# nwihardjo/SpaghettiSearch

Hardware: AMD Instinct MI355X
Metric: pagerank_iters_per_sec (higher is better)
Workload: dtype f64

## Files before the change

### spaghettisearch_amd/csrc/ctx.hip

```cpp
#include "common.hpp"
#include <chrono>

#include <unordered_map>

namespace ss {

namespace {
struct Pool {
    std::mutex mu;
    std::multimap<std::pair<int, size_t>, void*> free_blocks;
    std::unordered_map<void*, std::pair<int, size_t>> live;
    size_t held = 0, limit = (size_t)64 << 30;
    double miss_ms = 0.0;
    uint64_t misses = 0;
    int contexts = 0;
};
Pool& pool() { static Pool* p = new Pool(); return *p; }
size_t size_class(size_t b) {
    if (b <= 4096) return 4096;
    size_t p2 = 4096;
    while (p2 < b) p2 <<= 1;
    if (p2 <= ((size_t)1 << 20)) return p2;
    const size_t step = p2 >> 4;
    return (b + step - 1) / step * step;
}
}

hipError_t pool_alloc(void** out, size_t bytes) {
    Pool& P = pool();
    const size_t cls = size_class(bytes);
    int dev = 0;
    (void)hipGetDevice(&dev);
    {
        std::lock_guard<std::mutex> lk(P.mu);
        auto it = P.free_blocks.find({dev, cls});
        if (it != P.free_blocks.end()) {
            *out = it->second;
            P.free_blocks.erase(it);
            P.held -= cls;
            P.live[*out] = {dev, cls};
            return hipSuccess;
        }
    }
    const auto tm0 = std::chrono::steady_clock::now();
    hipError_t e = hipMalloc(out, cls);
    {
        std::lock_guard<std::mutex> lk(P.mu);
        P.miss_ms += std::chrono::duration<double, std::milli>(std::chrono::steady_clock::now() - tm0).count();
        P.misses++;
    }
    if (e != hipSuccess) {
        (void)hipGetLastError();
        pool_trim();
        e = hipMalloc(out, cls);
    }
    if (e == hipSuccess) {
        std::lock_guard<std::mutex> lk(P.mu);
        P.live[*out] = {dev, cls};
    }
    return e;
}

static thread_local bool t_device_idle = false;

void pool_free_batch(void* const* blocks, size_t count) {
    if (!count) return;
    {
        int cur = 0;
        (void)hipGetDevice(&cur);
        if (device_wedged(cur)) return;
    }
    (void)hipDeviceSynchronize();
    t_device_idle = true;
    for (size_t i = 0; i < count; i++) pool_free(blocks[i]);
    t_device_idle = false;
}

void pool_free(void* p) {
    if (!p) return;
    Pool& P = pool();
    size_t cls = 0, limit = 0;
    int dev = 0;
    {
        std::lock_guard<std::mutex> lk(P.mu);
        auto it = P.live.find(p);
        if (it != P.live.end()) { dev = it->second.first; cls = it->second.second; P.live.erase(it); }
        limit = P.limit;
    }
    if (device_wedged(dev)) return;
    if (cls && cls <= limit / 2) {
        int cur = 0;
        (void)hipGetDevice(&cur);
        if (cur != dev || !t_device_idle) {
            if (cur != dev) (void)hipSetDevice(dev);
            (void)hipDeviceSynchronize();
            if (cur != dev) (void)hipSetDevice(cur);
        }
        std::vector<void*> evict;
        {
            std::lock_guard<std::mutex> lk(P.mu);
            while (P.held + cls > P.limit && !P.free_blocks.empty()) {
                auto last = std::prev(P.free_blocks.end());
                if (last->first.second <= cls) break;
                evict.push_back(last->second);
                P.held -= last->first.second;
                P.free_blocks.erase(last);
            }
            if (P.held + cls <= P.limit) {
                P.free_blocks.emplace(std::make_pair(dev, cls), p);
                P.held += cls;
                p = nullptr;
            }
        }
        for (void* q : evict) (void)hipFree(q);
        if (!p) return;
    }
    (void)hipFree(p);
}

void pool_stats(uint64_t* misses, double* miss_ms) {
    std::lock_guard<std::mutex> lk(pool().mu);
    *misses = pool().misses;
    *miss_ms = pool().miss_ms;
}
void pool_context_count(int delta) {
    bool last = false;
    {
        std::lock_guard<std::mutex> lk(pool().mu);
        pool().contexts += delta;
        last = delta < 0 && pool().contexts <= 0;
    }
    if (last) pool_trim();
}

void pool_trim() {
    Pool& P = pool();
    std::multimap<std::pair<int, size_t>, void*> take;
    {
        std::lock_guard<std::mutex> lk(P.mu);
        take.swap(P.free_blocks);
        P.held = 0;
    }
    for (auto& kv : take) (void)hipFree(kv.second);
}

void pool_set_limit(size_t bytes) {
    {
        std::lock_guard<std::mutex> lk(pool().mu);
        pool().limit = bytes;
    }
    pool_trim();
}

static std::mutex g_err_mu;
static std::string g_err;
void set_global_error(const std::string& msg) {
    std::lock_guard<std::mutex> lk(g_err_mu);
    g_err = msg;
}
}

extern "C" {

int32_t ss_abi_version(void) { return SS_ABI_VERSION; }

int32_t ss_init(int32_t device_id, ss_ctx** out) {
    if (!out) {
        ss::set_global_error("ss_init: out is NULL");
        return SS_ERR_INVALID;
    }
    *out = nullptr;
    int n_dev = 0;
    hipError_t e = hipGetDeviceCount(&n_dev);
    if (e != hipSuccess || n_dev <= 0) {
        ss::set_global_error(std::string("ss_init: no HIP device (") + hipGetErrorString(e) + ")");
        return SS_ERR_NO_DEVICE;
    }
    if (device_id < 0 || device_id >= n_dev) {
        ss::set_global_error("ss_init: device_id out of range");
        return SS_ERR_INVALID;
    }
    ss_ctx* ctx = new (std::nothrow) ss_ctx();
    if (!ctx) return SS_ERR_OOM;
    ctx->device = device_id;
    if ((e = hipSetDevice(device_id)) != hipSuccess) {
        ss::set_global_error(std::string("ss_init: hipSetDevice: ") + hipGetErrorString(e));
        delete ctx;
        return SS_ERR_NO_DEVICE;
    }
    hipDeviceProp_t prop;
    if ((e = hipGetDeviceProperties(&prop, device_id)) != hipSuccess) {
        ss::set_global_error(std::string("ss_init: hipGetDeviceProperties: ") + hipGetErrorString(e));
        delete ctx;
        return SS_ERR_NO_DEVICE;
    }
    if (std::strncmp(prop.gcnArchName, "gfx950", 6) != 0) {
        ss::set_global_error(std::string("ss_init: device is ") + prop.gcnArchName +
                             ", this library is built for gfx950 (MI355X) only");
        delete ctx;
        return SS_ERR_NO_DEVICE;
    }
    ctx->cu_count = prop.multiProcessorCount;
    ctx->total_mem = prop.totalGlobalMem;
    if ((e = hipStreamCreateWithFlags(&ctx->own_stream, hipStreamNonBlocking)) != hipSuccess) {
        ss::set_global_error(std::string("ss_init: hipStreamCreate: ") + hipGetErrorString(e));
        delete ctx;
        return SS_ERR_HIP;
    }
    ctx->stream = ctx->own_stream;
    int prio_lo = 0, prio_hi = 0;
    (void)hipDeviceGetStreamPriorityRange(&prio_lo, &prio_hi);
    if ((e = hipStreamCreateWithPriority(&ctx->comm_stream, hipStreamNonBlocking, prio_hi)) != hipSuccess) {
        ss::set_global_error(std::string("ss_init: hipStreamCreate (comm): ") + hipGetErrorString(e));
        (void)hipStreamDestroy(ctx->own_stream);
        delete ctx;
        return SS_ERR_HIP;
    }
    for (int k = 0; k < 3; k++)
        for (int j = 0; j < 2; j++)
            if ((e = hipEventCreate(&ctx->ev[k][j])) != hipSuccess) {
                ss::set_global_error(std::string("ss_init: hipEventCreate: ") + hipGetErrorString(e));
                delete ctx;
                return SS_ERR_HIP;
            }
    if ((e = hipHostMalloc(reinterpret_cast<void**>(&ctx->h_pin), ss_ctx::PIN_SCRATCH, hipHostMallocDefault)) != hipSuccess) {
        ss::set_global_error(std::string("ss_init: hipHostMalloc: ") + hipGetErrorString(e));
        delete ctx;
        return SS_ERR_HIP;
    }
    ss::pool_context_count(+1);
    *out = ctx;
    return SS_OK;
}

int32_t ss_shutdown(ss_ctx* ctx) {
    if (!ctx) return SS_ERR_INVALID;
    (void)hipSetDevice(ctx->device);
    const bool stuck = !ss::try_unwedge(ctx);
    (void)ss_comm_destroy(ctx);
    if (!stuck) (void)hipStreamSynchronize(ctx->stream);
    for (int k = 0; k < 3; k++)
        for (int j = 0; j < 2; j++)
            if (ctx->ev[k][j]) (void)hipEventDestroy(ctx->ev[k][j]);
    if (ctx->comm_stream && !stuck) { (void)hipStreamSynchronize(ctx->comm_stream); (void)hipStreamDestroy(ctx->comm_stream); }
    for (hipStream_t ws : ctx->wave_stream)
        if (ws && !stuck) { (void)hipStreamSynchronize(ws); (void)hipStreamDestroy(ws); }
    if (ctx->own_stream && !stuck) (void)hipStreamDestroy(ctx->own_stream);
    if (ctx->h_pin) (void)hipHostFree(ctx->h_pin);
    for (auto& b : ctx->pin_cache) (void)hipHostFree(b.p);
    delete ctx;
    ss::pool_context_count(-1);
    return SS_OK;
}

int32_t ss_set_stream(ss_ctx* ctx, void* hip_stream) {
    if (!ctx) return SS_ERR_INVALID;
    std::lock_guard<std::recursive_mutex> lk(ctx->mu);
    SS_HIP(ctx, hipStreamSynchronize(ctx->stream));
    ctx->stream = hip_stream ? reinterpret_cast<hipStream_t>(hip_stream) : ctx->own_stream;
    return SS_OK;
}

static const char* const k_option_names[] = {
    "comm.timeout_ms",
    "pr.force_narrow",
    "pr.wire_f32",
    "pr.narrow_wave",
    "pr.t_quad",
    "pr.blocks_per_cu",
    "mem.pool_mb",
    "pr.deal_snake",
    "pr.affine_lag",
    "pr.affine",
    "pr.items_per_wave",
    "pr.persistent",
    "pr.persistent_blocks",
    "pr.n_class_order",
    "pr.class_order",
    "pr.stagger",
    "pr.deal_global",
    "pr.share_zero_rows",
    "pr.item_turns",
    "graph.late_free",
    "pr.trace",
    "score.collect_pinned",
    "score.pipeline_slices",
    "score.timing",
    "score.trace",
    "pr.probe_hot",
    "pr.topic_blocks",
    "tfidf.blocks",
    "tfidf.bucket_shift",
    "tfidf.head_min_run",
    "tfidf.bucket_min",
    "score.wave",
    "score.wave_max_terms",
    "score.wave_min_list",
    "score.wave_share_pct",
    "score.wave_slice_target",
    "score.wave_big_pct",
    "score.wave_big_x100",
    "score.small",
    "score.small_max_batch",
    "score.small_batch",
    "score.small_cap",
    "score.pipeline",
    "score.grade_slices",
    "score.wave_small_x100",
    "score.exact_all",
    "score.slice_target",
    "score.separate_merge",
};

int32_t ss_set_option(ss_ctx* ctx, const char* name, int64_t value) {
    if (!ctx || !name) return SS_ERR_INVALID;
    std::lock_guard<std::recursive_mutex> lk(ctx->mu);
    for (const char* n : k_option_names)
        if (std::strcmp(n, name) == 0) {
            if (value == SS_OPTION_DEFAULT) ctx->options.erase(name);
            else ctx->options[name] = value;
            if (std::strcmp(name, "mem.pool_mb") == 0) ss::pool_set_limit(value == SS_OPTION_DEFAULT ? (size_t)64 << 30 : (size_t)std::max<int64_t>(0, value) << 20);
            return SS_OK;
        }
    return ctx->fail(SS_ERR_INVALID, "ss_set_option: unknown option '%s'", name);
}

int32_t ss_synchronize(ss_ctx* ctx) {
    if (!ctx) return SS_ERR_INVALID;
    std::lock_guard<std::recursive_mutex> lk(ctx->mu);
    SS_HIP(ctx, hipSetDevice(ctx->device));
    SS_TRY(ss::sync_bounded(ctx, ctx->stream, "ss_synchronize"));
    return SS_OK;
}

const char* ss_last_error(ss_ctx* ctx) {
    if (ctx) return ctx->last_error.c_str();
    static thread_local std::string tl;
    {
        std::lock_guard<std::mutex> lk(ss::g_err_mu);
        tl = ss::g_err;
    }
    return tl.c_str();
}

int32_t ss_last_kernel_ms(ss_ctx* ctx, int32_t kind, float* ms_out) {
    if (!ctx || !ms_out || kind < 0 || kind > 2) return SS_ERR_INVALID;
    std::lock_guard<std::recursive_mutex> lk(ctx->mu);
    if (!ctx->ev_valid[kind]) return ctx->fail(SS_ERR_STATE, "ss_last_kernel_ms: no timed call of kind %d yet", kind);
    SS_HIP(ctx, hipEventSynchronize(ctx->ev[kind][1]));
    SS_HIP(ctx, hipEventElapsedTime(ms_out, ctx->ev[kind][0], ctx->ev[kind][1]));
    return SS_OK;
}

}
```

### spaghettisearch_amd/csrc/pagerank.hip

```cpp
#include "pr_device.hpp"

#include <algorithm>
#include <chrono>
#include <cmath>
#include <memory>

namespace {

__global__ void k_pr_item_ranges(WorkItem* __restrict__ work, uint32_t n_items, const uint32_t* __restrict__ in_ptr) {
    const uint32_t i = blockIdx.x * blockDim.x + threadIdx.x;
    if (i >= n_items) return;
    WorkItem w = work[i];
    switch (w.kind) {
        case V_ROWW: w.beg = in_ptr[w.row]; w.end = in_ptr[w.row + 1]; break;
        case V_SEG:
            w.beg = in_ptr[w.row] + w.count * SEGW;
            w.end = min(in_ptr[w.row + 1], w.beg + SEGW);
            break;
        case V_QUAD:
        case V_DEG: w.beg = in_ptr[w.row]; w.end = in_ptr[w.row + w.count]; break;
        default: return;
    }
    work[i] = w;
}

__global__ __launch_bounds__(TPB) void k_pr_remap_src(const uint32_t* __restrict__ in_src, uint32_t* __restrict__ out, size_t n_edges, uint32_t pos_nd,
                                                      uint32_t cnt_nd, const uint32_t* __restrict__ outdeg, const uint32_t* __restrict__ sh_deg,
                                                      uint32_t n_shared, uint32_t zrow) {
    for (size_t e = (size_t)blockIdx.x * TPB + threadIdx.x; e < n_edges; e += (size_t)gridDim.x * TPB) {
        uint32_t w = NT_LOAD(&in_src[e]);
        const uint32_t s = w & SRC_MASK;
        if (s >= pos_nd) {
            uint32_t row = zrow;
            if (s < cnt_nd && n_shared) {
                const uint32_t od = outdeg[s];
                uint32_t lo = 0, hi = n_shared;
                while (lo < hi) {
                    const uint32_t mid = (lo + hi) >> 1;
                    if (sh_deg[mid] < od) lo = mid + 1; else hi = mid;
                }
                if (lo < n_shared && sh_deg[lo] == od) row = zrow + 1 + lo;
            }
            w = (w & ~SRC_MASK) | row;
        }
        NT_STORE(w, &out[e]);
    }
}

template <int GW>
__global__ __launch_bounds__(TPB) void k_pr_begin(PrParams p) {
    const int lane = threadIdx.x & 63;
    const int t = lane % GW;
    const double x0 = p.x0[t];
    double* __restrict__ Tw = p.tab_wr[1];
    double csum = 0.0;
    for (uint32_t i = blockIdx.x * TPB + threadIdx.x; i < p.n_shared * (uint32_t)GW; i += gridDim.x * TPB)
        Tw[(size_t)(p.zrow + 1) * GW + i] = p.d * x0 / (double)p.sh_deg[i / GW];
    const size_t n_el = ((size_t)p.sl_nd + p.sl_d) * GW;
    for (size_t i = (size_t)blockIdx.x * TPB + threadIdx.x; i < n_el; i += (size_t)gridDim.x * TPB) {
        const uint32_t lrow = (uint32_t)(i / GW);
        const bool real = lrow < p.sl_nd ? lrow < p.cnt_nd : (lrow - p.sl_nd) < p.cnt_d;
        p.x[i] = real ? x0 : 0.0;
        if (lrow < p.sl_nd) {
            double c = 0.0;
            if (real) c = p.d * x0 / (double)p.outdeg[lrow];
            if ((p.world == 1 || lrow + 2 < p.sl_nd) && lrow < p.tab_rows) Tw[i] = c;
            csum += c;
        }
    }
    block_reduce_and_publish<GW>(p, 0.0, csum, Tw, true);
}

template <int GW>
__global__ void k_pr_finalize(PrParams p, const double* __restrict__ table, int is_begin) {
    if (threadIdx.x != 0 || blockIdx.x != 0) return;
    if (!is_begin && p.ctl->n_active == 0) return;
    double dl[MAXK], cs[MAXK];
    for (int k = 0; k < MAXK; k++) { dl[k] = 0.0; cs[k] = 0.0; }
    for (int r = 0; r < p.world; r++) {
        const size_t base = ((size_t)r * p.sl_nd + (p.sl_nd - 2)) * GW;
        for (int k = 0; k < GW; k++) {
            cs[k] += table[base + k];
            dl[k] += table[base + GW + k];
        }
    }
    finalize_ctl(p, dl, cs, is_begin != 0);
}

template <int GW>
__global__ void k_pr_read(const double* __restrict__ x, const PrCtl* __restrict__ ctl, const uint32_t* __restrict__ old_id,
                          uint32_t sl_nd, uint32_t cnt_nd, uint32_t pos_nd, uint32_t sl_d, uint32_t cnt_d, uint32_t pos_d,
                          uint64_t id0_nd, uint64_t id0_d, int k_topics, uint64_t out_stride,
                          int by_original_id, uint32_t* __restrict__ ids_out, double* __restrict__ out,
                          const uint32_t* __restrict__ memb, uint32_t ts_mask) {
    const size_t n_rows = (size_t)cnt_nd + cnt_d;
    size_t i = (size_t)blockIdx.x * blockDim.x + threadIdx.x;
    if (i >= n_rows) return;
    const uint32_t lrow = i < cnt_nd ? (uint32_t)i : sl_nd + (uint32_t)(i - cnt_nd);
    const uint64_t iid = lrow < sl_nd ? id0_nd + lrow : id0_d + (lrow - sl_nd);
    const uint32_t orig = old_id[iid];
    const size_t o = by_original_id ? (size_t)orig : i;
    if (ids_out) ids_out[i] = orig;
    const bool zero = lrow < sl_nd ? lrow >= pos_nd : (lrow - sl_nd) >= pos_d;
    const uint32_t mb = memb ? memb[lrow] & ts_mask : 0u;
    for (int k = 0; k < k_topics; k++)
        out[(size_t)k * out_stride + o] = zero ? (((mb >> k) & 1u) ? ctl->xz_in[k] : ctl->xz[k]) : x[(size_t)lrow * GW + k];
}

__global__ void k_pr_memb(const uint64_t* __restrict__ set_ptr, const uint32_t* __restrict__ set_nodes, int k_topics, uint64_t n_nodes,
                          const uint32_t* __restrict__ new_id, uint64_t nd_int, uint32_t sl_nd, uint32_t sl_d, int rank,
                          uint32_t* __restrict__ memb, uint32_t* __restrict__ seen, uint32_t* __restrict__ err) {
    const uint64_t total = set_ptr[k_topics];
    for (uint64_t i = (uint64_t)blockIdx.x * blockDim.x + threadIdx.x; i < total; i += (uint64_t)gridDim.x * blockDim.x) {
        int k = 0;
        while (k + 1 < k_topics && set_ptr[k + 1] <= i) k++;
        const uint32_t v = set_nodes[i];
        if ((uint64_t)v >= n_nodes) { atomicOr(err, 1u); continue; }
        if (atomicOr(&seen[v], 1u << k) & (1u << k)) { atomicOr(err, 2u); continue; }
        const uint64_t iid = new_id[v];
        uint32_t lrow;
        int owner;
        if (iid < nd_int) { owner = (int)(iid / sl_nd); lrow = (uint32_t)(iid % sl_nd); }
        else { owner = (int)((iid - nd_int) / sl_d); lrow = sl_nd + (uint32_t)((iid - nd_int) % sl_d); }
        if (owner == rank) atomicOr(&memb[lrow], 1u << k);
    }
}
__global__ void k_pr_memb_zero_count(const uint32_t* __restrict__ memb, uint32_t sl_nd, uint32_t cnt_nd, uint32_t pos_nd, uint32_t cnt_d,
                                     uint32_t pos_d, int k_topics, unsigned long long* __restrict__ cnt) {
    const uint32_t z_nd = cnt_nd - pos_nd, n_zero = z_nd + (cnt_d - pos_d);
    for (uint32_t i = blockIdx.x * blockDim.x + threadIdx.x; i < n_zero; i += gridDim.x * blockDim.x) {
        const uint32_t lrow = i < z_nd ? pos_nd + i : sl_nd + pos_d + (i - z_nd);
        const uint32_t mb = memb[lrow];
        for (int k = 0; k < k_topics; k++)
            if ((mb >> k) & 1u) atomicAdd(&cnt[k], 1ull);
    }
}

template <int GW, int POL>
__global__ __launch_bounds__(TPB) void k_pr_probe(const double* __restrict__ T, const uint32_t* __restrict__ in_src, size_t n_edges,
                                                  uint32_t n_rows, int mode, double* __restrict__ sink, uint32_t hot) {
    if constexpr (GW >= 8) {
        constexpr int NSLOT = 64 / GW;
        const int lane = threadIdx.x & 63, wave = threadIdx.x >> 6;
        const int t = lane % GW, slot = lane / GW, gbase = lane - t;
        const size_t groups = (size_t)gridDim.x * WAVES * NSLOT;
        const size_t gi = ((size_t)blockIdx.x * WAVES + wave) * NSLOT + slot;
        const size_t n_chunks = n_edges / CH;
        const size_t per = (n_chunks + groups - 1) / groups;
        size_t c = min(gi * per, n_chunks);
        const size_t c_hi = min(c + per, n_chunks);
        double acc = 0.0;
        for (; c < c_hi; c++) {
            constexpr int R = CH / GW;
            uint32_t src[R];
#pragma unroll
            for (int r = 0; r < R; r++) {
                const size_t e = c * CH + (size_t)(r * GW + t);
                uint32_t v = NT_LOAD(&in_src[e]) & SRC_MASK;
                if (mode == 1) v = (uint32_t)(((uint64_t)(v * 2654435761u + (uint32_t)e * 40503u) * n_rows) >> 32);
                if (mode == 2) v = (uint32_t)(e % n_rows);
                src[r] = v;
            }
            double v[CH];
#pragma unroll
            for (int j = 0; j < CH; j++) {
                const uint32_t sj = (uint32_t)__shfl((int)src[j / GW], gbase + (j % GW), 64);
                const double* a = &T[(size_t)sj * GW + t];
                if constexpr (POL == 0) v[j] = *a;
                else if constexpr (POL == 1) v[j] = __builtin_nontemporal_load(a);
                else if constexpr (POL == 2) v[j] = __hip_atomic_load(a, __ATOMIC_RELAXED, __HIP_MEMORY_SCOPE_AGENT);
                else if constexpr (POL == 3) v[j] = sj < hot ? *a : __builtin_nontemporal_load(a);
                else v[j] = sj < hot ? *a : __hip_atomic_load(a, __ATOMIC_RELAXED, __HIP_MEMORY_SCOPE_AGENT);
            }
#pragma unroll
            for (int j = 0; j < CH; j++) acc += v[j];
        }
        sink[((size_t)blockIdx.x * TPB + threadIdx.x)] = acc;
    }
}

}

namespace {

void pick_kernel(const ss_ctx* ctx, ss_pr* pr, int k, uint64_t table_rows) {
    const bool force_narrow = ctx->opt("pr.force_narrow", 0) != 0, narrow_wave = ctx->opt("pr.narrow_wave", 1) != 0;
    if (k > 2) {
        pr->kernel = PR_SWEEP;
        pr->gw = k <= 8 ? 8 : 16;
    } else if (force_narrow) {
        pr->kernel = PR_STEP;
        pr->gw = k;
    } else if (narrow_wave) {
        pr->kernel = PR_SWEEP_N;
        pr->gw = k;
    } else if (table_rows * 64 <= (64ull << 20)) {
        pr->kernel = PR_SWEEP;
        pr->gw = 8;
    } else {
        pr->kernel = PR_STEP;
        pr->gw = k;
    }
    pr->nwave = pr->kernel == PR_SWEEP_N;
    const int64_t want = ctx->opt("pr.persistent", 0);
    pr->persist_mode = want == 2 ? 2 : 1;
    pr->persist = pr->nwave && pr->g->world == 1 && !ctx->opt("pr.affine", 0) && want > 0;
}

template <int GW>
void launch_begin(ss_pr* pr, hipStream_t st, unsigned nb) {
    hipLaunchKernelGGL(k_pr_begin<GW>, dim3(nb), dim3(TPB), 0, st, pr->prm);
}
template <int GW>
void launch_finalize(ss_pr* pr, hipStream_t st, int is_begin) {
    hipLaunchKernelGGL(k_pr_finalize<GW>, dim3(1), dim3(64), 0, st, pr->prm, (const double*)pr->tab0.p, is_begin);
}
template <int GW>
__global__ __launch_bounds__(TPB) void k_pr_read_orig(const double* __restrict__ x, const PrCtl* __restrict__ ctl, const uint32_t* __restrict__ new_id,
                                                      uint64_t n, uint32_t sl_nd, uint32_t pos_nd, uint32_t pos_d, int k_topics,
                                                      double* __restrict__ out, const uint32_t* __restrict__ memb, uint32_t ts_mask) {
    const uint64_t v = (uint64_t)blockIdx.x * blockDim.x + threadIdx.x;
    if (v >= n) return;
    const uint32_t lrow = new_id[v];
    const bool zero = lrow < sl_nd ? lrow >= pos_nd : (lrow - sl_nd) >= pos_d;
    double r[GW];
    if (!zero) {
        if constexpr (GW >= 2) {
            const double2* const row = reinterpret_cast<const double2*>(x + (size_t)lrow * GW);
#pragma unroll
            for (int j = 0; j < GW / 2; j++) { const double2 t = row[j]; r[2 * j] = t.x; r[2 * j + 1] = t.y; }
        } else {
            r[0] = x[lrow];
        }
    } else {
        const uint32_t mb = memb ? memb[lrow] & ts_mask : 0u;
#pragma unroll
        for (int k = 0; k < GW; k++) r[k] = ((mb >> k) & 1u) ? ctl->xz_in[k] : ctl->xz[k];
    }
#pragma unroll
    for (int k = 0; k < GW; k++)
        if (k < k_topics) out[(size_t)k * n + v] = r[k];
}

template <int GW>
void launch_read(ss_pr* pr, hipStream_t st, int by_orig, uint64_t stride, uint32_t* ids, double* out) {
    const ss_graph* g = pr->g;
    const size_t n_rows = (size_t)g->cnt_nd + g->cnt_d;
    if (!n_rows) return;
    if (by_orig && g->world == 1 && !ids && stride == g->n) {
        hipLaunchKernelGGL(k_pr_read_orig<GW>, dim3(ss::div_up(g->n, TPB)), dim3(TPB), 0, st, (const double*)pr->x.p, (const PrCtl*)pr->ctl.p,
                           (const uint32_t*)g->new_id.p, g->n, g->sl_nd, pr->prm.pos_nd, pr->prm.pos_d, pr->k, out, pr->prm.memb, pr->prm.ts_mask);
        return;
    }
    hipLaunchKernelGGL(k_pr_read<GW>, dim3(ss::div_up(n_rows, TPB)), dim3(TPB), 0, st, (const double*)pr->x.p,
                       (const PrCtl*)pr->ctl.p, (const uint32_t*)g->old_id.p, g->sl_nd, g->cnt_nd, pr->prm.pos_nd, g->sl_d, g->cnt_d,
                       pr->prm.pos_d,
                       (uint64_t)g->rank * g->sl_nd, g->nd_int + (uint64_t)g->rank * g->sl_d, pr->k, stride, by_orig, ids, out,
                       pr->prm.memb, pr->prm.ts_mask);
}

#define SS_GW_DISPATCH(gw, fn, ...)          \
    switch (gw) {                            \
        case 1: fn<1>(__VA_ARGS__); break;   \
        case 2: fn<2>(__VA_ARGS__); break;   \
        case 8: fn<8>(__VA_ARGS__); break;   \
        default: fn<16>(__VA_ARGS__); break; \
    }

}

namespace ss {
unsigned begin_blocks(const ss_pr* pr) { return std::max(1u, std::min(2048u, ss::div_up((size_t)pr->g->n_local() * pr->gw, TPB))); }
void pr_launch_begin(ss_pr* pr, hipStream_t st, unsigned nb) { SS_GW_DISPATCH(pr->gw, launch_begin, pr, st, nb); }
void pr_launch_step(ss_pr* pr, hipStream_t st) {
    switch (pr->kernel) {
        case PR_STEP: pr_step_launch(pr, st); break;
        case PR_SWEEP: pr_sweep_launch(pr, st); break;
        case PR_SWEEP_N: pr_sweep_n_launch(pr, st); break;
    }
}
void pr_launch_finalize(ss_pr* pr, hipStream_t st, int is_begin) { SS_GW_DISPATCH(pr->gw, launch_finalize, pr, st, is_begin); }
}

namespace {

PlanOptions plan_options(const ss_ctx* ctx, const ss_pr* pr, size_t n_local) {
    const bool small = n_local <= ((size_t)4 << 20);
    PlanOptions o;
    o.t_quad = (uint32_t)ctx->opt("pr.t_quad", pr->nwave ? 256 : 128);
    o.item_turns = (uint32_t)std::max<int64_t>(1, std::min<int64_t>(64, ctx->opt("pr.item_turns", pr->nwave ? (small ? 1 : 4) : (small ? 4 : 8))));
    o.items_per_wave = pr->nwave ? (size_t)std::max<int64_t>(1, ctx->opt("pr.items_per_wave", 4)) : 1;
    o.deal_snake = ctx->opt("pr.deal_snake", PlanOptions::AUTO);
    o.deal_global = ctx->opt("pr.deal_global", pr->nwave && pr->gw == 1 ? 1 : 2);
    o.blocks_per_cu = ctx->opt("pr.blocks_per_cu", PlanOptions::AUTO);
    o.class_order = ctx->opt("pr.class_order", 235401);
    o.n_class_order = ctx->opt("pr.n_class_order", small ? 2310 : 123);
    o.stagger = ctx->opt("pr.stagger", 0);
    return o;
}

constexpr int OCC_MULTI_N = 3;
int blocks_per_cu(int row, int gw) {
    static std::mutex occ_mu;
    static int occ_cache[4][MAXK + 1] = {};
    std::lock_guard<std::mutex> lk_occ(occ_mu);
    int& occ = occ_cache[row][gw];
    if (!occ) {
        int per_cu = 0;
        switch (row) {
            case PR_STEP: per_cu = ss::pr_step_occupancy(gw); break;
            case PR_SWEEP: per_cu = ss::pr_sweep_occupancy(gw); break;
            case PR_SWEEP_N: per_cu = ss::pr_sweep_n_occupancy(gw); break;
            default: per_cu = ss::pr_multi_n_occupancy(gw); break;
        }
        occ = std::max(per_cu, 1);
    }
    return occ;
}
unsigned grid_for(const ss_ctx* ctx, const ss_pr* pr, const PlanOptions& opt, int per_cu, size_t n_items) {
    per_cu = (int)std::max<int64_t>(1, opt.blocks_per_cu == PlanOptions::AUTO ? per_cu : opt.blocks_per_cu);
    if (pr->persist) {
        const int admit = std::max(1, blocks_per_cu(OCC_MULTI_N, pr->gw) - 2);
        per_cu = (int)std::max<int64_t>(1, std::min<int64_t>(std::min(admit, std::max(1, per_cu / 2)), ctx->opt("pr.persistent_blocks", 4)));
    }
    return pr->kernel != PR_STEP ? (unsigned)std::min<size_t>(std::max<size_t>(1, ss::div_up(n_items, (size_t)WAVES * opt.items_per_wave)), (size_t)ctx->cu_count * per_cu)
                                 : (unsigned)std::min<size_t>(n_items, (size_t)ctx->cu_count * 8);
}

void fill_params(ss_pr* pr, const Cut& cut, const PlanOptions& opt, double damping, double eps, int32_t max_iter, int32_t k_topics) {
    const ss_graph* g = pr->g;
    PrParams& p = pr->prm;
    p.in_ptr = g->in_ptr.p;
    p.in_src = g->in_src.p;
    p.outdeg = g->outdeg.p;
    p.x = pr->x.p;
    if (g->world == 1) {
        p.tab_rd[0] = pr->tab0.p; p.tab_wr[0] = pr->tab1.p;
        p.tab_rd[1] = pr->tab1.p; p.tab_wr[1] = pr->tab0.p;
    } else {
        p.tab_rd[0] = p.tab_rd[1] = pr->tab0.p;
        p.tab_wr[0] = p.tab_wr[1] = pr->send.p;
    }
    p.work = pr->work.p;
    p.partials = pr->partials.p;
    p.segpart = pr->segpart.p;
    p.rowticket = pr->rowticket.p;
    p.ctl = pr->ctl.p;
    p.x0 = pr->x0.p;
    p.d = damping;
    p.teleport = 1.0 - damping;
    p.eps = eps;
    p.tele_n = p.teleport * (double)g->n;
    p.max_iter = max_iter;
    p.k_topics = k_topics;
    p.world = g->world;
    p.sl_nd = g->sl_nd;
    p.cnt_nd = g->cnt_nd;
    p.sl_d = g->sl_d;
    p.cnt_d = g->cnt_d;
    p.seg_edges = cut.seg_edges;
    p.n_items = (uint32_t)cut.items.size();
    p.pos_nd = cut.pos_nd;
    p.pos_d = cut.pos_d;
    p.zrow = (uint32_t)g->nd_int;
    p.tab_rows = g->sl_nd;
    p.woff = pr->woff.p;
    p.stagger_div = opt.stagger != 0 ? (uint32_t)std::max(g->ctx->cu_count, 1) : 0u;
    p.stagger_code = opt.stagger >= 10 ? (uint32_t)(opt.stagger - 10) : 0u;
    p.class_order = pack_class_order(opt.class_order);
    p.n_order = pack_n_order(opt.n_class_order);
}

uint64_t fnv1a(const void* q, size_t n, uint64_t h = 0xcbf29ce484222325ull) {
    const unsigned char* b = static_cast<const unsigned char*>(q);
    for (size_t i = 0; i < n; i++) { h ^= b[i]; h *= 0x100000001b3ull; }
    return h;
}
void trace_plan(const ss_pr* pr, const std::vector<WorkItem>& work, const std::vector<uint32_t>& woff) {
    const PrParams& p = pr->prm;
    const double sd[] = {p.d, p.teleport, p.eps, p.tele_n};
    const uint32_t su[] = {(uint32_t)p.max_iter, (uint32_t)p.k_topics, (uint32_t)p.world, p.sl_nd, p.cnt_nd, p.sl_d, p.cnt_d, p.seg_edges, p.n_items,
                           p.pos_nd, p.pos_d, p.ts_mask, p.zrow, p.stagger_div, p.stagger_code, p.class_order, p.n_order};
    fprintf(stderr, "[pr trace] plan: work %016llx (%zu items)  woff %016llx  params %016llx  nblocks %u\n",
            (unsigned long long)fnv1a(work.data(), work.size() * sizeof(WorkItem)), work.size(),
            (unsigned long long)fnv1a(woff.data(), woff.size() * sizeof(uint32_t)),
            (unsigned long long)fnv1a(su, sizeof(su), fnv1a(sd, sizeof(sd))), pr->nblocks);
}

int32_t alloc_tables(ss_pr* pr, hipStream_t st, size_t rows) {
    const ss_graph* g = pr->g;
    ss_ctx* ctx = g->ctx;
    const size_t GW = (size_t)pr->gw;
    SS_HIP(ctx, pr->tab0.alloc(rows * GW));
    SS_HIP(ctx, hipMemsetAsync(pr->tab0.p, 0, std::max<size_t>(pr->tab0.bytes(), 8), st));
    if (g->world == 1) {
        SS_HIP(ctx, pr->tab1.alloc(rows * GW));
        SS_HIP(ctx, hipMemsetAsync(pr->tab1.p, 0, std::max<size_t>(pr->tab1.bytes(), 8), st));
    } else {
        SS_HIP(ctx, pr->send.alloc((size_t)g->sl_nd * GW));
        SS_HIP(ctx, hipMemsetAsync(pr->send.p, 0, std::max<size_t>(pr->send.bytes(), 8), st));
    }
    return SS_OK;
}
int32_t unshare_rows(ss_pr* pr, hipStream_t st) {
    if (!pr->prm.share) return SS_OK;
    const ss_graph* g = pr->g;
    SS_HIP(g->ctx, hipStreamSynchronize(st));
    SS_TRY(alloc_tables(pr, st, (size_t)g->nd_int + 1));
    pr->src_shared.release();
    pr->sh_deg.release();
    PrParams& p = pr->prm;
    p.tab_rd[0] = pr->tab0.p; p.tab_wr[0] = pr->tab1.p;
    p.tab_rd[1] = pr->tab1.p; p.tab_wr[1] = pr->tab0.p;
    p.in_src = g->in_src.p;
    p.sh_deg = nullptr;
    p.n_shared = 0;
    p.share = 0;
    p.zrow = (uint32_t)g->nd_int;
    p.tab_rows = g->sl_nd;
    return SS_OK;
}

#ifdef SS_PR_WAVETIME
void dump_wave_loads(const Cut& cut, const std::vector<double>& cost, const std::vector<uint32_t>& owner, uint32_t nw) {
    FILE* f = open_dump("pr_load.csv");
    if (!f) return;
    std::vector<double> wl(nw, 0.0), wcls((size_t)nw * 6, 0.0);
    for (size_t i = 0; i < cut.items.size(); i++) {
        int kc = 0; while (kc < 5 && i >= cut.vbeg[kc + 1]) kc++;
        wl[owner[i]] += cost[i]; wcls[(size_t)owner[i] * 6 + kc] += cost[i];
    }
    fprintf(f, "wave,load,c0,c1,c2,c3,c4,c5\n");
    for (uint32_t w = 0; w < nw; w++) fprintf(f, "%u,%.2f,%.2f,%.2f,%.2f,%.2f,%.2f,%.2f\n", w, wl[w], wcls[(size_t)w * 6], wcls[(size_t)w * 6 + 1], wcls[(size_t)w * 6 + 2], wcls[(size_t)w * 6 + 3], wcls[(size_t)w * 6 + 4], wcls[(size_t)w * 6 + 5]);
    fclose(f);
}
#endif

}

extern "C" {

int32_t ss_pr_create(ss_graph* g, double damping, double eps, int32_t max_iter, int32_t k_topics,
                     const int32_t* n_topic, ss_pr** out) {
    if (!g) return SS_ERR_INVALID;
    ss_ctx* ctx = g->ctx;
    std::lock_guard<std::recursive_mutex> lk(ctx->mu);
    if (!out) return ctx->fail(SS_ERR_INVALID, "ss_pr_create: out is NULL");
    *out = nullptr;
    if (k_topics < 1 || !n_topic) return ctx->fail(SS_ERR_INVALID, "ss_pr_create: k_topics < 1 or n_topic NULL");
    if (k_topics > MAXK) return ctx->fail(SS_ERR_UNSUPPORTED, "ss_pr_create: k_topics %d > %d per state (ss_pagerank_run splits larger K)", k_topics, MAXK);
    SS_HIP(ctx, hipSetDevice(ctx->device));
    hipStream_t st = ctx->stream;

    ss_pr* pr = new (std::nothrow) ss_pr();
    if (!pr) return ctx->fail(SS_ERR_OOM, "ss_pr_create: host OOM");
    std::unique_ptr<ss_pr> guard(pr);
    pr->g = g;
    pr->k = k_topics;
    pick_kernel(ctx, pr, k_topics, g->nd_int);
    const int GW = pr->gw;
    const bool vitems = pr->kernel != PR_STEP;
    const int GI = pr->nwave ? 8 : GW;
    const size_t n_local = g->n_local();
    if (((uint64_t)g->nd_int + 1) * GW * 8 >= (1ull << 32))
        return ctx->fail(SS_ERR_UNSUPPORTED, "ss_pr_create: contribution table of %llu rows x %d topics exceeds 4 GiB (shard the graph over more ranks)",
                         (unsigned long long)g->nd_int, GW);

    const bool trace = ctx->opt("pr.trace", 0) != 0;
    auto t_now = [] { return std::chrono::steady_clock::now(); };
    auto t_ms = [](std::chrono::steady_clock::time_point a, std::chrono::steady_clock::time_point b) { return std::chrono::duration<double, std::milli>(b - a).count(); };
    SS_HIP(ctx, pr->x.alloc(n_local * GW));
    bool share = GW >= 8 && g->world == 1 && ctx->opt("pr.affine", 0) == 0 && ctx->opt("pr.share_zero_rows", 1) != 0;
    if (!share) SS_TRY(alloc_tables(pr, st, (size_t)g->nd_int + 1));

    const auto tc0 = t_now();
    const PlanOptions opt = plan_options(ctx, pr, n_local);
    Cut cut = cut_items(g->h_indeg_nd, g->h_indeg_d, g->sl_nd, GI, pr->nwave, opt);
    const uint32_t n_tail = g->cnt_nd - cut.pos_nd;
    struct PinGuard { ss_ctx* c; void* p = nullptr; size_t cap = 0; ~PinGuard() { c->pin_free(p, cap); } } tail_od{ctx};
    if (share && n_tail == 0) {
        share = false;
        SS_TRY(alloc_tables(pr, st, (size_t)g->nd_int + 1));
    }
    if (share) {
        tail_od.p = ctx->pin_alloc((size_t)n_tail * sizeof(uint32_t), &tail_od.cap);
        if (!tail_od.p) return ctx->fail(SS_ERR_OOM, "ss_pr_create: no pinned host memory for %u out-degrees", n_tail);
        SS_HIP(ctx, hipMemcpyAsync(tail_od.p, g->outdeg.p + cut.pos_nd, (size_t)n_tail * sizeof(uint32_t), hipMemcpyDeviceToHost, st));
    }
    const auto tc1 = t_now();
    const int per_cu = blocks_per_cu(pr->kernel, GW);
    const auto tc1a = t_now();
    pr->nblocks = grid_for(ctx, pr, opt, per_cu, cut.items.size());
    static const std::vector<uint32_t> no_woff;
    const std::vector<uint32_t>* woff = &no_woff;
    if (vitems) {
        const uint32_t nw = pr->nblocks * WAVES;
        const auto td0 = t_now();
        const std::vector<double>& cost = item_costs(cut, g->h_indeg_nd, g->h_indeg_d, g->sl_nd, GI, pr->nwave);
        const auto td0a = t_now();
        std::vector<uint32_t>& owner = deal_items(cut, cost, nw, pr->nwave, opt);
#ifdef SS_PR_WAVETIME
        dump_wave_loads(cut, cost, owner, nw);
#endif
        const auto td1 = t_now();
        if (trace) fprintf(stderr, "[pr trace]   deal: occupancy query %.2f ms, costs %.3f ms, owners %.3f ms\n", t_ms(tc1, tc1a), t_ms(td0, td0a), t_ms(td0a, td1));
        woff = &place_items(cut, owner, nw);
        if (trace) fprintf(stderr, "[pr trace]   deal: placement %.3f ms\n", t_ms(td1, t_now()));
    }
    const std::vector<WorkItem>& items = cut.items;

    g->settle();
    const auto tc2 = t_now();
    SharedRows sh;
    if (share) {
        SS_HIP(ctx, hipStreamSynchronize(st));
        const auto ts0 = t_now();
        sh = plan_shared_rows(static_cast<const uint32_t*>(tail_od.p), n_tail, cut.pos_nd);
        const auto ts1 = t_now();
        SS_TRY(alloc_tables(pr, st, (size_t)sh.table_rows));
        SS_HIP(ctx, pr->sh_deg.alloc(sh.deg.size()));
        SS_HIP(ctx, hipMemcpyAsync(pr->sh_deg.p, sh.deg.data(), sh.deg.size() * sizeof(uint32_t), hipMemcpyHostToDevice, st));
        SS_HIP(ctx, pr->src_shared.alloc(g->e_local));
        if (g->e_local)
            hipLaunchKernelGGL(k_pr_remap_src, dim3((unsigned)std::min<uint64_t>(ss::div_up(g->e_local, TPB), (uint64_t)ctx->cu_count * 16)), dim3(TPB), 0, st,
                               (const uint32_t*)g->in_src.p, pr->src_shared.p, (size_t)g->e_local, cut.pos_nd, g->cnt_nd, (const uint32_t*)g->outdeg.p,
                               (const uint32_t*)pr->sh_deg.p, (uint32_t)sh.deg.size(), sh.zrow);
        if (trace) fprintf(stderr, "[pr trace]   shared rows: %u rows without in-edges -> %zu shared rows (host %.3f ms), table %llu rows\n", n_tail, sh.deg.size(),
                           t_ms(ts0, ts1), (unsigned long long)sh.table_rows);
    }
    SS_HIP(ctx, pr->partials.alloc(((size_t)std::max(pr->nblocks, ss::begin_blocks(pr)) + 8) * 2 * GW));
    SS_HIP(ctx, pr->segpart.alloc((size_t)std::max(cut.nsegs, 1u) * GW));
    SS_HIP(ctx, pr->rowticket.alloc(std::max(cut.nmulti, 1u)));
    SS_HIP(ctx, hipMemsetAsync(pr->rowticket.p, 0, pr->rowticket.bytes(), st));
    SS_HIP(ctx, pr->woff.alloc(std::max<size_t>(woff->size(), 8)));
    if (!woff->empty()) SS_HIP(ctx, hipMemcpyAsync(pr->woff.p, woff->data(), woff->size() * sizeof(uint32_t), hipMemcpyHostToDevice, st));
    SS_HIP(ctx, pr->work.alloc(items.size()));
    SS_HIP(ctx, hipMemcpyAsync(pr->work.p, items.data(), items.size() * sizeof(WorkItem), hipMemcpyHostToDevice, st));
    if (vitems)
        hipLaunchKernelGGL(k_pr_item_ranges, dim3(ss::div_up(items.size(), TPB)), dim3(TPB), 0, st, pr->work.p, (uint32_t)items.size(), (const uint32_t*)g->in_ptr.p);
    SS_HIP(ctx, pr->ctl.alloc(1));
    SS_HIP(ctx, hipMemsetAsync(pr->ctl.p, 0, sizeof(PrCtl), st));
    double h_x0[MAXK];
    for (int k = 0; k < MAXK; k++) h_x0[k] = k < k_topics ? 1.0 / (double)n_topic[k] : 0.0;
    SS_HIP(ctx, pr->x0.alloc(MAXK));
    SS_HIP(ctx, hipMemcpyAsync(pr->x0.p, h_x0, sizeof(h_x0), hipMemcpyHostToDevice, st));
    SS_HIP(ctx, hipStreamSynchronize(st));
    if (trace) fprintf(stderr, "[pr trace] ss_pr_create: build_work %.2f ms (%zu items), edge ranges + deal %.2f ms, alloc + upload %.2f ms\n", t_ms(tc0, tc1), items.size(), t_ms(tc1, tc2), t_ms(tc2, t_now()));
    if (trace) fprintf(stderr, "[pr trace] where the state lives: x %p  tab0 %p  tab1 %p  in_src %p  in_ptr %p  outdeg %p  work %p  woff %p\n", (void*)pr->x.p, (void*)pr->tab0.p,
                       (void*)pr->tab1.p, (void*)g->in_src.p, (void*)g->in_ptr.p, (void*)g->outdeg.p, (void*)pr->work.p, (void*)pr->woff.p);

    fill_params(pr, cut, opt, damping, eps, max_iter, k_topics);
    if (share) {
        PrParams& p = pr->prm;
        p.in_src = pr->src_shared.p;
        p.sh_deg = pr->sh_deg.p;
        p.n_shared = (uint32_t)sh.deg.size();
        p.share = 1;
        p.zrow = sh.zrow;
        p.tab_rows = cut.pos_nd;
    }
    if (trace) trace_plan(pr, items, *woff);
    g->users++;
    *out = guard.release();
    return SS_OK;
}

int32_t ss_pr_set_teleport(ss_pr* pr, const uint64_t* set_ptr, const uint32_t* set_nodes) {
    if (!pr) return SS_ERR_INVALID;
    ss_ctx* ctx = pr->g->ctx;
    std::lock_guard<std::recursive_mutex> lk(ctx->mu);
    SS_HIP(ctx, hipSetDevice(ctx->device));
    if (pr->begun) return ctx->fail(SS_ERR_STATE, "ss_pr_set_teleport: call before ss_pr_begin");
    hipStream_t st = ctx->stream;
    PrParams& p = pr->prm;
    if (!set_ptr) {
        p.memb = nullptr; p.tin = nullptr; p.nz_in = nullptr; p.ts_mask = 0;
        return SS_OK;
    }
    const ss_graph* g = pr->g;
    const int K = pr->k;
    SS_TRY(unshare_rows(pr, st));
    std::vector<uint64_t> h_ptr(K + 1);
    SS_HIP(ctx, ss::copy_in(ctx->stream, h_ptr.data(), set_ptr, (K + 1) * sizeof(uint64_t)));
    if (h_ptr[0] != 0) return ctx->fail(SS_ERR_INVALID, "ss_pr_set_teleport: set_ptr[0] != 0");
    for (int k = 0; k < K; k++)
        if (h_ptr[k + 1] < h_ptr[k]) return ctx->fail(SS_ERR_INVALID, "ss_pr_set_teleport: set_ptr not non-decreasing");
    const uint64_t total = h_ptr[K];
    if (total && !set_nodes) return ctx->fail(SS_ERR_INVALID, "ss_pr_set_teleport: set_nodes is NULL");
    double h_tin[MAXK];
    uint32_t mask = 0;
    for (int k = 0; k < MAXK; k++) {
        h_tin[k] = 0.0;
        if (k < K && h_ptr[k + 1] > h_ptr[k]) {
            mask |= 1u << k;
            h_tin[k] = p.teleport * (double)g->n / (double)(h_ptr[k + 1] - h_ptr[k]);
        }
    }
    const size_t n_local = g->n_local();
    ss::DevBuf<uint64_t> d_ptr;
    ss::DevBuf<uint32_t> d_nodes, d_err, d_seen;
    ss::DevBuf<unsigned long long> d_cnt;
    SS_HIP(ctx, d_ptr.alloc(K + 1));
    SS_HIP(ctx, d_seen.alloc(g->n));
    SS_HIP(ctx, hipMemsetAsync(d_seen.p, 0, std::max<size_t>(d_seen.bytes(), 4), st));
    SS_HIP(ctx, d_nodes.alloc(total));
    SS_HIP(ctx, d_err.alloc(1));
    SS_HIP(ctx, d_cnt.alloc(MAXK));
    SS_HIP(ctx, pr->memb.alloc(n_local));
    SS_HIP(ctx, pr->tin.alloc(MAXK));
    SS_HIP(ctx, pr->nz_in.alloc(MAXK));
    SS_HIP(ctx, hipMemcpyAsync(d_ptr.p, h_ptr.data(), (K + 1) * sizeof(uint64_t), hipMemcpyHostToDevice, st));
    if (total) SS_HIP(ctx, hipMemcpyAsync(d_nodes.p, set_nodes, total * sizeof(uint32_t), hipMemcpyDefault, st));
    SS_HIP(ctx, hipMemsetAsync(pr->memb.p, 0, std::max<size_t>(pr->memb.bytes(), 4), st));
    SS_HIP(ctx, hipMemsetAsync(d_err.p, 0, sizeof(uint32_t), st));
    SS_HIP(ctx, hipMemsetAsync(d_cnt.p, 0, MAXK * sizeof(unsigned long long), st));
    if (total)
        hipLaunchKernelGGL(k_pr_memb, dim3(std::min<unsigned>(ss::div_up(total, TPB), 4096u)), dim3(TPB), 0, st, (const uint64_t*)d_ptr.p,
                           (const uint32_t*)d_nodes.p, K, g->n, (const uint32_t*)g->new_id.p, g->nd_int, std::max(g->sl_nd, 1u), std::max(g->sl_d, 1u),
                           g->rank, pr->memb.p, d_seen.p, d_err.p);
    const uint32_t n_zero = (g->cnt_nd - p.pos_nd) + (g->cnt_d - p.pos_d);
    if (n_zero)
        hipLaunchKernelGGL(k_pr_memb_zero_count, dim3(std::min<unsigned>(ss::div_up(n_zero, TPB), 4096u)), dim3(TPB), 0, st,
                           (const uint32_t*)pr->memb.p, g->sl_nd, g->cnt_nd, p.pos_nd, g->cnt_d, p.pos_d, K, d_cnt.p);
    SS_HIP(ctx, hipGetLastError());
    uint32_t h_err = 0;
    unsigned long long h_cnt[MAXK];
    SS_HIP(ctx, ss::fetch(ctx, st, &h_err, d_err.p, sizeof(h_err), h_cnt, d_cnt.p, sizeof(h_cnt)));
    if (h_err & 1u) return ctx->fail(SS_ERR_INVALID, "ss_pr_set_teleport: a teleport set holds a node id >= n_nodes");
    if (h_err & 2u) return ctx->fail(SS_ERR_INVALID, "ss_pr_set_teleport: a teleport set lists a node twice (the ids of a set must be distinct)");
    double h_nz[MAXK];
    for (int k = 0; k < MAXK; k++) h_nz[k] = (double)h_cnt[k];
    SS_HIP(ctx, hipMemcpyAsync(pr->tin.p, h_tin, sizeof(h_tin), hipMemcpyHostToDevice, st));
    SS_HIP(ctx, hipMemcpyAsync(pr->nz_in.p, h_nz, sizeof(h_nz), hipMemcpyHostToDevice, st));
    SS_HIP(ctx, hipStreamSynchronize(st));
    p.memb = pr->memb.p;
    p.tin = pr->tin.p;
    p.nz_in = pr->nz_in.p;
    p.ts_mask = mask;
    return SS_OK;
}

int32_t ss_pr_destroy(ss_pr* pr) {
#ifdef SS_PR_WAVETIME
    if (pr) ss::pr_dump_wave_times(pr);
#endif

    if (!pr) return SS_ERR_INVALID;
    ss_ctx* ctx = pr->g->ctx;
    std::lock_guard<std::recursive_mutex> lk(ctx->mu);
    (void)hipSetDevice(ctx->device);
    if (!ss::device_wedged(ctx->device)) {
        (void)hipStreamSynchronize(ctx->stream);
        (void)hipStreamSynchronize(ctx->comm_stream);
    }
    pr->g->users--;
    delete pr;
    return SS_OK;
}

int32_t ss_pr_begin(ss_pr* pr) {
    if (!pr) return SS_ERR_INVALID;
    ss_ctx* ctx = pr->g->ctx;
    std::lock_guard<std::recursive_mutex> lk(ctx->mu);
    SS_HIP(ctx, hipSetDevice(ctx->device));
    if (pr->need_finalize) return ctx->fail(SS_ERR_STATE, "ss_pr_begin: pending exchange/finalize");
    SS_HIP(ctx, hipMemsetAsync(&pr->ctl.p->ticket, 0, sizeof(uint32_t), ctx->stream));
    ss::pr_launch_begin(pr, ctx->stream, ss::begin_blocks(pr));
    SS_HIP(ctx, hipGetLastError());
    pr->begun = true;
    if (pr->g->world > 1) {
        pr->need_finalize = true;
        pr->finalize_is_begin = true;
    }
    return SS_OK;
}

int32_t ss_pr_step(ss_pr* pr, int32_t n_steps) {
    if (!pr) return SS_ERR_INVALID;
    ss_ctx* ctx = pr->g->ctx;
    std::lock_guard<std::recursive_mutex> lk(ctx->mu);
    SS_HIP(ctx, hipSetDevice(ctx->device));
    if (!pr->begun) return ctx->fail(SS_ERR_STATE, "ss_pr_step: ss_pr_begin not called");
    if (pr->need_finalize) return ctx->fail(SS_ERR_STATE, "ss_pr_step: pending exchange/finalize");
    if (n_steps < 1) return ctx->fail(SS_ERR_INVALID, "ss_pr_step: n_steps < 1");
    if (pr->g->world > 1 && n_steps != 1) return ctx->fail(SS_ERR_INVALID, "ss_pr_step: world>1 needs an exchange after every step");
    SS_HIP(ctx, hipEventRecord(ctx->ev[0][0], ctx->stream));
    if (pr->persist && !pr->prm.memb && !pr->prm.aff) {
        ss::pr_multi_n_launch(pr, ctx->stream, (int)n_steps);
    } else {
        for (int i = 0; i < n_steps; i++) ss::pr_launch_step(pr, ctx->stream);
    }
    SS_HIP(ctx, hipEventRecord(ctx->ev[0][1], ctx->stream));
    ctx->ev_valid[0] = true;
    SS_HIP(ctx, hipGetLastError());
    if (pr->g->world > 1) {
        pr->need_finalize = true;
        pr->finalize_is_begin = false;
    }
    return SS_OK;
}

int32_t ss_pr_finalize(ss_pr* pr) {
    if (!pr) return SS_ERR_INVALID;
    ss_ctx* ctx = pr->g->ctx;
    std::lock_guard<std::recursive_mutex> lk(ctx->mu);
    SS_HIP(ctx, hipSetDevice(ctx->device));
    if (pr->g->world == 1) return ctx->fail(SS_ERR_STATE, "ss_pr_finalize: world==1 folds the finalize into the sweep");
    if (!pr->need_finalize) return ctx->fail(SS_ERR_STATE, "ss_pr_finalize: nothing to finalize");
    ss::pr_launch_finalize(pr, ctx->stream, pr->finalize_is_begin ? 1 : 0);
    SS_HIP(ctx, hipGetLastError());
    pr->need_finalize = false;
    return SS_OK;
}

int32_t ss_pr_exchange_buffers(ss_pr* pr, void** send_dev, uint64_t* send_bytes, void** recv_dev, uint64_t* recv_bytes) {
    if (!pr) return SS_ERR_INVALID;
    ss_ctx* ctx = pr->g->ctx;
    if (pr->g->world == 1) return ctx->fail(SS_ERR_STATE, "ss_pr_exchange_buffers: world==1 has no exchange");
    if (send_dev) *send_dev = pr->send.p;
    if (send_bytes) *send_bytes = pr->send.bytes();
    if (recv_dev) *recv_dev = pr->tab0.p;
    if (recv_bytes) *recv_bytes = (uint64_t)pr->g->nd_int * pr->gw * sizeof(double);
    return SS_OK;
}

int32_t ss_pr_exchange(ss_pr* pr, int32_t allreduce) {
    if (!pr) return SS_ERR_INVALID;
    ss_ctx* ctx = pr->g->ctx;
    std::lock_guard<std::recursive_mutex> lk(ctx->mu);
    SS_HIP(ctx, hipSetDevice(ctx->device));
    const ss_graph* g = pr->g;
    if (g->world == 1) return ctx->fail(SS_ERR_STATE, "ss_pr_exchange: world==1 has no exchange");
    if (!pr->need_finalize) return ctx->fail(SS_ERR_STATE, "ss_pr_exchange: nothing to exchange (call after ss_pr_begin / ss_pr_step)");
    if (!ctx->comm || ctx->comm_world != g->world || ctx->comm_rank != g->rank)
        return ctx->fail(SS_ERR_STATE, "ss_pr_exchange: the context's communicator (rank %d of %d) does not match the graph's shard (rank %d of %d)",
                         ctx->comm ? ctx->comm_rank : -1, ctx->comm ? ctx->comm_world : 0, g->rank, g->world);
    const size_t slice = (size_t)g->sl_nd * pr->gw;
    if (!allreduce && ctx->opt("pr.wire_f32", 0) != 0) {
        SS_HIP(ctx, ss::pr_wire_alloc(pr));
        ss::pr_wire_pack(pr, ctx->stream);
        SS_TRY(ss::comm_allgather(ctx, pr->wire_send.p, pr->wire_recv.p, ss::pr_wire_floats(pr) * sizeof(float)));
        ss::pr_wire_unpack(pr, ctx->stream);
        return SS_OK;
    }
    if (!allreduce) return ss::comm_allgather(ctx, pr->send.p, pr->tab0.p, slice * sizeof(double));
    SS_HIP(ctx, hipMemsetAsync(pr->tab0.p, 0, pr->tab0.bytes(), ctx->stream));
    SS_HIP(ctx, hipMemcpyAsync(pr->tab0.p + (size_t)g->rank * slice, pr->send.p, slice * sizeof(double), hipMemcpyDeviceToDevice, ctx->stream));
    return ss::comm_allreduce_f64(ctx, pr->tab0.p, pr->tab0.p, slice * (size_t)g->world);
}

int32_t ss_pr_status(ss_pr* pr, int32_t* iters_out, int32_t* n_active, int32_t* sweeps, double* last_delta_out,
                     double* last_total_out) {
    if (!pr) return SS_ERR_INVALID;
    ss_ctx* ctx = pr->g->ctx;
    std::lock_guard<std::recursive_mutex> lk(ctx->mu);
    SS_HIP(ctx, hipSetDevice(ctx->device));
    const PrCtl* hp = nullptr;
    SS_TRY(read_ctl(ctx, pr, ctx->stream, "ss_pr_status", &hp));
    const PrCtl h = *hp;
    if (h.stuck) return ctx->fail(SS_ERR_STATE, "ss_pr_status: the multi-sweep kernel gave up waiting between two sweeps (its grid of %u blocks was not resident: "
                                  "other kernels held the CUs for seconds); the state is void — set option pr.persistent = 0 and run again", pr->nblocks);
    for (int k = 0; k < pr->k; k++) {
        if (iters_out) iters_out[k] = h.iters[k];
        if (last_delta_out) last_delta_out[k] = h.delta[k];
        if (last_total_out) last_total_out[k] = h.S[k];
    }
    if (n_active) *n_active = h.n_active;
    if (sweeps) *sweeps = h.sweep;
    return SS_OK;
}

int32_t ss_pr_read_local(ss_pr* pr, uint32_t* ids_out, double* rank_out) {
    if (!pr || !rank_out) return SS_ERR_INVALID;
    ss_ctx* ctx = pr->g->ctx;
    std::lock_guard<std::recursive_mutex> lk(ctx->mu);
    SS_HIP(ctx, hipSetDevice(ctx->device));
    const ss_graph* g = pr->g;
    const size_t n_rows = (size_t)g->cnt_nd + g->cnt_d;
    ss::DevBuf<uint32_t> d_ids;
    ss::DevBuf<double> d_out;
    SS_HIP(ctx, d_ids.alloc(n_rows));
    SS_HIP(ctx, d_out.alloc(n_rows * pr->k));
    SS_GW_DISPATCH(pr->gw, launch_read, pr, ctx->stream, 0, (uint64_t)n_rows, d_ids.p, d_out.p);
    SS_HIP(ctx, hipGetLastError());
    if (ids_out && n_rows) SS_HIP(ctx, hipMemcpyAsync(ids_out, d_ids.p, n_rows * sizeof(uint32_t), hipMemcpyDefault, ctx->stream));
    if (n_rows) SS_HIP(ctx, hipMemcpyAsync(rank_out, d_out.p, n_rows * pr->k * sizeof(double), hipMemcpyDefault, ctx->stream));
    SS_HIP(ctx, hipStreamSynchronize(ctx->stream));
    return SS_OK;
}

int32_t ss_pr_read(ss_pr* pr, double* rank_out) {
    if (!pr || !rank_out) return SS_ERR_INVALID;
    ss_ctx* ctx = pr->g->ctx;
    std::lock_guard<std::recursive_mutex> lk(ctx->mu);
    SS_HIP(ctx, hipSetDevice(ctx->device));
    const ss_graph* g = pr->g;
    if (g->world != 1) return ctx->fail(SS_ERR_STATE, "ss_pr_read: world>1, use ss_pr_read_local");
    hipPointerAttribute_t pa{};
    const bool dev_out = hipPointerGetAttributes(&pa, rank_out) == hipSuccess && pa.type == hipMemoryTypeDevice;
    (void)hipGetLastError();
    ss::DevBuf<double> d_out;
    if (!dev_out) SS_HIP(ctx, d_out.alloc((size_t)g->n * pr->k));
    SS_GW_DISPATCH(pr->gw, launch_read, pr, ctx->stream, 1, (uint64_t)g->n, (uint32_t*)nullptr, dev_out ? rank_out : d_out.p);
    SS_HIP(ctx, hipGetLastError());
    if (!dev_out) SS_HIP(ctx, hipMemcpyAsync(rank_out, d_out.p, (size_t)g->n * pr->k * sizeof(double), hipMemcpyDefault, ctx->stream));
    SS_HIP(ctx, hipStreamSynchronize(ctx->stream));
    return SS_OK;
}

int32_t ss_pr_probe(ss_pr* pr, int32_t mode, int32_t n_reps, float* ms_out) {
    if (!pr || !ms_out) return SS_ERR_INVALID;
    ss_ctx* ctx = pr->g->ctx;
    std::lock_guard<std::recursive_mutex> lk(ctx->mu);
    SS_HIP(ctx, hipSetDevice(ctx->device));
    if (pr->gw < 8) return ctx->fail(SS_ERR_UNSUPPORTED, "ss_pr_probe: the probe mirrors the chunked gather of the K >= 5 kernels");
    if (mode < 0 || (mode & 7) > 2 || (mode >> 3) > 4 || n_reps < 1) return ctx->fail(SS_ERR_INVALID, "ss_pr_probe: mode 0..2 (+ 8 * gather cache policy 0..4), n_reps >= 1");
    const int pol = mode >> 3;
    mode &= 7;
    const uint32_t hot = (uint32_t)ctx->opt("pr.probe_hot", 24576);
    const ss_graph* g = pr->g;
    const unsigned nb = (unsigned)ctx->cu_count * 8;
    ss::DevBuf<double> sink;
    SS_HIP(ctx, sink.alloc((size_t)nb * TPB));
    hipEvent_t e0, e1;
    SS_HIP(ctx, hipEventCreate(&e0));
    SS_HIP(ctx, hipEventCreate(&e1));
    hipStream_t st = ctx->stream;
    ss::DevBuf<double> full;
    if (pr->prm.share) {
        SS_HIP(ctx, full.alloc(((size_t)g->nd_int + 1) * pr->gw));
        SS_HIP(ctx, hipMemsetAsync(full.p, 0, full.bytes(), ctx->stream));
    }
    const double* T = pr->prm.share ? full.p : pr->tab0.p;
    for (int r = 0; r < n_reps + 1; r++) {
        if (r == 1) SS_HIP(ctx, hipEventRecord(e0, st));
#define SS_PROBE_LAUNCH(GWV, POLV) hipLaunchKernelGGL((k_pr_probe<GWV, POLV>), dim3(nb), dim3(TPB), 0, st, T, (const uint32_t*)g->in_src.p, (size_t)g->e_local, (uint32_t)g->nd_int, mode, sink.p, hot)
        if (pr->gw == 8) SS_PROBE_LAUNCH(8, 0);
        else switch (pol) {
            case 0: SS_PROBE_LAUNCH(16, 0); break;
            case 1: SS_PROBE_LAUNCH(16, 1); break;
            case 2: SS_PROBE_LAUNCH(16, 2); break;
            case 3: SS_PROBE_LAUNCH(16, 3); break;
            default: SS_PROBE_LAUNCH(16, 4); break;
        }
    }
    SS_HIP(ctx, hipEventRecord(e1, st));
    SS_HIP(ctx, hipEventSynchronize(e1));
    float ms = 0.f;
    SS_HIP(ctx, hipEventElapsedTime(&ms, e0, e1));
    (void)hipEventDestroy(e0);
    (void)hipEventDestroy(e1);
    SS_HIP(ctx, hipGetLastError());
    *ms_out = ms / (float)n_reps;
    return SS_OK;
}

}
```

### spaghettisearch_amd/csrc/pr_plan.hpp

```cpp
#pragma once
#include "sorted_degrees.hpp"

#include <algorithm>
#include <cstdint>
#include <utility>
#include <vector>

namespace {

constexpr int TPB = 256;
constexpr int WAVES = TPB / 64;
constexpr int CH = 16;
constexpr uint32_t SEGW = 2048;

enum : uint32_t { W_SEG = 0, W_WAVE = 1, W_GROUP = 2, W_ZERO = 3,
                  V_SEG = 8,
                  V_ROWW = 9,
                  V_QUAD = 10,
                  V_DEG = 11,
                  V_ZERO = 12 };

struct WorkItem {
    uint32_t kind;
    uint32_t row;
    uint32_t count;
    uint32_t nseg;
    uint32_t sbase;
    uint32_t tix;
    uint32_t beg, end;
};

constexpr uint32_t plan_div_up(uint64_t a, uint64_t b) { return (uint32_t)((a + b - 1) / b); }

struct PlanOptions {
    static constexpr int64_t AUTO = INT64_MIN;
    uint32_t t_quad = 128;
    uint32_t item_turns = 4;
    size_t items_per_wave = 1;
    int64_t deal_snake = AUTO;
    int64_t deal_global = 2;
    int64_t blocks_per_cu = AUTO;
    int64_t class_order = 235401;
    int64_t n_class_order = 2310;
    int64_t stagger = 0;
};

struct PlanScratch {
    std::vector<WorkItem> seg, rwg, wav, grp, zer;
    std::vector<WorkItem> vseg, vroww, vquad, vdeg[3], vzero;
    std::vector<WorkItem> items, dealt;
    std::vector<double> cost, load;
    std::vector<uint32_t> owner, by_load, idx, order, bucket, woff, cnt;
    std::vector<std::pair<double, uint32_t>> key;
};
inline PlanScratch& plan_scratch() {
    static thread_local PlanScratch s;
    return s;
}

struct Cut {
    std::vector<WorkItem>& items;
    uint32_t nsegs = 0, nmulti = 0;
    uint32_t seg_edges = 0;
    uint32_t pos_nd = 0, pos_d = 0;
    uint32_t vbeg[7] = {0};
};

inline Cut cut_items(const ss::SortedDegrees& nd, const ss::SortedDegrees& d, uint32_t sl_nd, int gw, bool lane_rows, const PlanOptions& opt) {
    PlanScratch& s = plan_scratch();
    Cut cut{s.items};
    uint32_t& nsegs = cut.nsegs;
    uint32_t& nmulti = cut.nmulti;
    const uint32_t NSLOT = 64 / gw;
    const uint32_t T_SEG = 32 * NSLOT;
    const uint32_t T_WAVE = 2 * NSLOT;
    const uint32_t seg_edges = cut.seg_edges = 128 * NSLOT;
    auto &seg = s.seg, &rwg = s.rwg, &wav = s.wav, &grp = s.grp, &zer = s.zer;
    auto &vseg = s.vseg, &vroww = s.vroww, &vquad = s.vquad, &vzero = s.vzero;
    auto& vdeg = s.vdeg;
    for (auto* v : {&seg, &rwg, &wav, &grp, &zer, &vseg, &vroww, &vquad, &vdeg[0], &vdeg[1], &vdeg[2], &vzero}) v->clear();
    auto emit_v = [&](const ss::SortedDegrees& deg, uint32_t row0, bool non_dangling, uint32_t& n_pos) {
        const uint32_t cnt = (uint32_t)deg.size();
        const uint32_t T_MULTI = 4096, T_DEG = 8;
        const uint32_t T_QUAD = opt.t_quad;
        const uint32_t item_turns = opt.item_turns;
        size_t j_at = 0, j_lim = 0;
        const size_t n_run = deg.val.size();
        auto deg_at = [&](uint32_t r) -> uint32_t {
            while (deg.start[j_at + 1] <= r) j_at++;
            return deg.val[j_at];
        };
        auto end_above = [&](uint32_t lim) -> uint32_t {
            while (j_lim < n_run && deg.val[j_lim] > lim) j_lim++;
            return deg.start[j_lim];
        };
        uint32_t r = 0;
        for (; r < cnt && deg_at(r) > T_MULTI; r++) {
            const uint32_t ns = (deg_at(r) + SEGW - 1) / SEGW;
            const uint32_t tix = nmulti++;
            for (uint32_t sg = 0; sg < ns; sg++) vseg.push_back({V_SEG, row0 + r, sg, ns, nsegs, tix});
            nsegs += ns;
        }
        {
            const uint32_t end = std::min(cnt, end_above(T_QUAD));
            for (; r < end; r++) vroww.push_back({V_ROWW, row0 + r, 0, 0, 0, 0});
        }
        while (r < cnt && deg_at(r) > T_DEG) {
            const uint32_t nch = (deg_at(r) + CH - 1) / CH;
            const uint32_t max_groups = std::min<uint32_t>((uint32_t)gw, std::max<uint32_t>(1u, 2u * item_turns / nch));
            const uint32_t lim = std::max<uint32_t>(T_DEG, (nch - 1) * CH);
            const uint32_t end = end_above(lim);
            const uint32_t same = end > r ? end - r : 0u;
            const uint32_t rows = std::min<uint32_t>(same, max_groups * NSLOT);
            vquad.push_back({V_QUAD, row0 + r, rows, nch, 0, 0});
            r += rows;
        }
        while (r < cnt && deg_at(r) > 0) {
            const uint32_t D = deg_at(r);
            const uint32_t run = deg.start[j_at + 1] - r;
            const uint32_t R = D <= 2 ? 8 : D <= 4 ? 4 : 2;
            const uint32_t per_item = lane_rows ? 64u * item_turns : NSLOT * R * item_turns;
            auto& out = vdeg[R == 2 ? 0 : R == 4 ? 1 : 2];
            for (uint32_t o = 0; o < run; o += per_item) out.push_back({V_DEG, row0 + r + o, std::min(per_item, run - o), D, 0, 0});
            r += run;
        }
        n_pos = r;
        const uint32_t ZERO_ROWS = 16 * NSLOT;
        if (non_dangling)
            for (uint32_t o = r; o < cnt; o += ZERO_ROWS) vzero.push_back({V_ZERO, row0 + o, std::min<uint32_t>(ZERO_ROWS, cnt - o), 0, 0, 0});
    };
    auto emit = [&](const ss::SortedDegrees& deg, uint32_t row0, bool non_dangling, uint32_t& n_pos) {
        if (gw >= 8) { emit_v(deg, row0, non_dangling, n_pos); return; }
        const uint32_t cnt = (uint32_t)deg.size();
        const uint32_t a = deg.first_at_most(T_SEG);
        const uint32_t c = std::max(a, deg.first_at_most(0));
        for (uint32_t r = 0; r < a; r++) {
            const uint32_t ns = (deg[r] + seg_edges - 1) / seg_edges;
            const uint32_t tix = ns > 1 ? nmulti++ : 0;
            for (uint32_t sg = 0; sg < ns; sg++) seg.push_back({W_SEG, row0 + r, sg, ns, nsegs, tix});
            nsegs += ns;
        }
        {
            const uint32_t b = std::min(c, std::max(a, deg.first_at_most(T_WAVE)));
            for (uint32_t r = a; r < b; r += WAVES) wav.push_back({W_WAVE, row0 + r, std::min<uint32_t>(WAVES, b - r), 0, 0, 0});
            const uint32_t GROUP_ROWS = WAVES * NSLOT * 4;
            for (uint32_t r = b; r < c; r += GROUP_ROWS) grp.push_back({W_GROUP, row0 + r, std::min<uint32_t>(GROUP_ROWS, c - r), 0, 0, 0});
        }
        n_pos = c;
        const uint32_t ZERO_ROWS = (TPB * 8) / gw;
        if (non_dangling)
            for (uint32_t r = c; r < cnt; r += ZERO_ROWS) zer.push_back({W_ZERO, row0 + r, std::min<uint32_t>(ZERO_ROWS, cnt - r), 0, 0, 0});
    };
    emit(nd, 0, true, cut.pos_nd);
    const size_t vquad_split = vquad.size();
    emit(d, sl_nd, false, cut.pos_d);
    auto& items = cut.items;
    auto& vbeg = cut.vbeg;
    items.clear();
    items.reserve(seg.size() + rwg.size() + wav.size() + grp.size() + zer.size());
    items.insert(items.end(), seg.begin(), seg.end());
    items.insert(items.end(), rwg.begin(), rwg.end());
    items.insert(items.end(), wav.begin(), wav.end());
    items.insert(items.end(), grp.begin(), grp.end());
    items.insert(items.end(), zer.begin(), zer.end());
    vbeg[0] = (uint32_t)items.size();
    items.insert(items.end(), vseg.begin(), vseg.end());
    items.insert(items.end(), vroww.begin(), vroww.end());
    vbeg[1] = (uint32_t)items.size();
    std::inplace_merge(vquad.begin(), vquad.begin() + (ptrdiff_t)vquad_split, vquad.end(),
                       [](const WorkItem& a, const WorkItem& b) { return a.nseg > b.nseg; });
    items.insert(items.end(), vquad.begin(), vquad.end());
    for (int k = 0; k < 3; k++) {
        vbeg[2 + k] = (uint32_t)items.size();
        items.insert(items.end(), vdeg[k].begin(), vdeg[k].end());
    }
    vbeg[5] = (uint32_t)items.size();
    items.insert(items.end(), vzero.begin(), vzero.end());
    vbeg[6] = (uint32_t)items.size();
    if (items.empty()) items.push_back({W_ZERO, 0, 0, 0, 0, 0});
    return cut;
}

inline const std::vector<double>& item_costs(const Cut& cut, const ss::SortedDegrees& nd, const ss::SortedDegrees& d, uint32_t sl_nd, int gw, bool lane_rows) {
    const std::vector<WorkItem>& items = cut.items;
    std::vector<double>& cost = plan_scratch().cost;
    const uint32_t NS = 64 / gw;
    struct DegCursor {
        const ss::SortedDegrees* d;
        size_t j = 0;
        uint32_t at(uint32_t r) {
            if (r >= d->size()) return 0u;
            if (d->start[j] > r) j = d->run_of(r);
            while (d->start[j + 1] <= r) j++;
            return d->val[j];
        }
    } cur_nd{&nd}, cur_d{&d};
    auto deg_of = [&](uint32_t lrow) -> uint32_t { return lrow < sl_nd ? cur_nd.at(lrow) : cur_d.at(lrow - sl_nd); };
    cost.assign(items.size(), 0.0);
    for (size_t i = 0; i < items.size(); i++) {
        const WorkItem& w = items[i];
        double turns = 1.0;
        switch (w.kind) {
            case V_ROWW: turns = plan_div_up(deg_of(w.row), NS * CH); break;
            case V_SEG: turns = plan_div_up(std::min<uint32_t>(SEGW, deg_of(w.row) - w.count * SEGW), NS * CH) + 2.0; break;
            case V_QUAD: turns = (double)plan_div_up(w.count, NS) * w.nseg; break;
            case V_DEG: {
                if (lane_rows) { turns = (double)plan_div_up(w.count, 64u) * (0.6 + 0.2 * (w.nseg <= 2 ? 2 : w.nseg <= 4 ? 4 : 8)); break; }
                const uint32_t R = w.nseg <= 2 ? 8 : w.nseg <= 4 ? 4 : 2;
                turns = (double)plan_div_up(w.count, NS * R) * (R == 8 ? 2.5 : R == 4 ? 1.7 : 1.3);
                break;
            }
            default: turns = 0.5; break;
        }
        cost[i] = turns + 1.0;
    }
    return cost;
}

inline std::vector<uint32_t>& deal_items(const Cut& cut, const std::vector<double>& cost, uint32_t nw, bool lane_rows, const PlanOptions& opt) {
    PlanScratch& s = plan_scratch();
    const size_t n_items = cut.items.size();
    auto &owner = s.owner, &by_load = s.by_load, &idx = s.idx, &order = s.order, &bucket = s.bucket;
    auto& load = s.load;
    auto& key = s.key;
    owner.assign(n_items, 0u);
    load.assign(nw, 0.0);
    by_load.resize(nw);
    for (uint32_t w = 0; w < nw; w++) by_load[w] = w;
    const bool snake = (opt.deal_snake == PlanOptions::AUTO ? (n_items >= (size_t)8 * nw || lane_rows ? 1 : 0) : opt.deal_snake) != 0;
    const int64_t deal_mode = opt.deal_global;
    const bool global_order = deal_mode != 0;
    if (global_order) {
        constexpr uint32_t NB = 1u << 14;
        const auto bkey = [&](size_t i) { return NB - 1 - (uint32_t)std::min<double>(cost[i] * 16.0, (double)(NB - 1)); };
        bucket.assign(NB + 1, 0u);
        order.resize(n_items);
        size_t c0 = 0;
        for (int kcls = 0; kcls < (deal_mode == 2 ? 6 : 1); kcls++) {
            const size_t c1 = deal_mode == 2 ? (kcls < 5 ? std::min<size_t>(cut.vbeg[kcls + 1], n_items) : n_items) : n_items;
            if (kcls) std::fill(bucket.begin(), bucket.end(), 0u);
            for (size_t i = c0; i < c1; i++) bucket[bkey(i) + 1]++;
            for (uint32_t b = 0; b < NB; b++) bucket[b + 1] += bucket[b];
            for (size_t i = c0; i < c1; i++) order[c0 + bucket[bkey(i)]++] = (uint32_t)i;
            c0 = c1;
        }
    }
    for (size_t i0 = 0; i0 < n_items; i0 += nw) {
        const size_t n_chunk = std::min<size_t>(nw, n_items - i0);
        if (i0 && snake) {
            std::reverse(by_load.begin(), by_load.end());
        } else if (i0) {
            key.resize(nw);
            for (uint32_t w = 0; w < nw; w++) key[w] = {load[w], w};
            std::sort(key.begin(), key.end());
            for (uint32_t w = 0; w < nw; w++) by_load[w] = key[w].second;
        }
        idx.resize(n_chunk);
        for (size_t j = 0; j < n_chunk; j++) idx[j] = global_order ? order[i0 + j] : (uint32_t)(i0 + j);
        const auto falling = [&](uint32_t a, uint32_t b) { return cost[a] > cost[b]; };
        size_t run_end = 0, n_merge = 0;
        for (size_t j = 1; j <= n_chunk && !global_order; j++) {
            if (j < n_chunk && !(cost[i0 + j] > cost[i0 + j - 1])) continue;
            if (run_end) {
                if (++n_merge > 8) { std::stable_sort(idx.begin(), idx.end(), falling); break; }
                std::inplace_merge(idx.begin(), idx.begin() + (ptrdiff_t)run_end, idx.begin() + (ptrdiff_t)j, falling);
            }
            run_end = j;
        }
        for (size_t j = 0; j < n_chunk; j++) {
            owner[idx[j]] = by_load[j];
            load[by_load[j]] += cost[idx[j]];
        }
    }
    return owner;
}

inline const std::vector<uint32_t>& place_items(Cut& cut, std::vector<uint32_t>& owner, uint32_t nw) {
    PlanScratch& s = plan_scratch();
    auto& items = cut.items;
    auto &woff = s.woff, &cnt = s.cnt;
    woff.assign((size_t)nw * 8, 0);
    cnt.assign((size_t)nw * 8, 0);
    for (int k = 0; k < 6; k++) {
        const size_t i1 = k < 5 ? std::min<size_t>(cut.vbeg[k + 1], items.size()) : items.size();
        for (size_t i = std::min<size_t>(cut.vbeg[k], i1); i < i1; i++) { owner[i] = owner[i] * 8 + (uint32_t)k; cnt[owner[i]]++; }
    }
    uint32_t run_off = 0;
    for (uint32_t w = 0; w < nw; w++) {
        for (int k = 0; k < 8; k++) {
            woff[(size_t)w * 8 + k] = run_off;
            run_off += cnt[(size_t)w * 8 + k];
            cnt[(size_t)w * 8 + k] = woff[(size_t)w * 8 + k];
        }
    }
    s.dealt.resize(items.size());
    for (size_t i = 0; i < items.size(); i++) s.dealt[cnt[owner[i]]++] = items[i];
    s.dealt.push_back({V_ZERO, 0, 0, 0, 0, 0, 0, 0});
    s.dealt.push_back({V_ZERO, 0, 0, 0, 0, 0, 0, 0});
    items.swap(s.dealt);
    return woff;
}

inline uint32_t pack_class_order(int64_t code) {
    uint32_t packed = 0, seen = 0;
    for (int pos = 5; pos >= 0; pos--) {
        const uint32_t c = (uint32_t)(code % 10);
        code /= 10;
        packed |= (c & 7u) << (3 * pos);
        if (c < 6) seen |= 1u << c;
    }
    return seen == 0x3Fu ? packed : (0u | 1u << 3 | 2u << 6 | 3u << 9 | 4u << 12 | 5u << 15);
}
inline uint32_t pack_n_order(int64_t code) {
    uint32_t packed = 0, seen = 0;
    for (int pos = 3; pos >= 0; pos--) {
        const uint32_t c = (uint32_t)(code % 10);
        code /= 10;
        packed |= (c & 3u) << (2 * pos);
        if (c < 4) seen |= 1u << c;
    }
    return seen == 0xFu ? packed : (0u | 1u << 2 | 2u << 4 | 3u << 6);
}

struct SharedRows {
    std::vector<uint32_t> deg;
    uint32_t zrow = 0;
    uint32_t base = 0;
    uint64_t table_rows = 0;
    uint32_t row_of(uint32_t od) const {
        const auto it = std::lower_bound(deg.begin(), deg.end(), od);
        return it != deg.end() && *it == od ? base + (uint32_t)(it - deg.begin()) : zrow;
    }
};
inline SharedRows plan_shared_rows(const uint32_t* od, size_t n, uint32_t pos_nd) {
    SharedRows sh;
    uint32_t hi = 0;
    for (size_t i = 0; i < n; i++) hi = std::max(hi, od[i]);
    if (n && (uint64_t)hi <= 4 * (uint64_t)n + 65536) {
        std::vector<unsigned char> seen((size_t)hi + 1, 0);
        for (size_t i = 0; i < n; i++) seen[od[i]] = 1;
        for (size_t v = 0; v <= hi; v++)
            if (seen[v]) sh.deg.push_back((uint32_t)v);
    } else if (n) {
        sh.deg.assign(od, od + n);
        std::sort(sh.deg.begin(), sh.deg.end());
        sh.deg.erase(std::unique(sh.deg.begin(), sh.deg.end()), sh.deg.end());
    }
    sh.zrow = pos_nd;
    sh.base = pos_nd + 1;
    sh.table_rows = (uint64_t)pos_nd + 1 + sh.deg.size();
    return sh;
}

}
```

### spaghettisearch_amd/csrc/pr_state.hpp

```cpp
#pragma once
#include "graph.hpp"
#include "pr_plan.hpp"

#ifdef SS_PR_WAVETIME
#include <cstdio>
#include <cstdlib>
#include <string>
#endif

namespace {

constexpr int MAXK = 16;

struct PrCtl {
    double S[MAXK];
    double delta[MAXK];
    double csum[MAXK];
    double xz[MAXK];
    double xz_in[MAXK];
    double tele[MAXK];
    int32_t active[MAXK];
    int32_t iters[MAXK];
    int32_t sweep;
    int32_t n_active;
    uint32_t ticket;
    uint32_t stuck;
    uint32_t gticket[8];
};

constexpr int AFF_MAXK = 256;
constexpr unsigned AFF_NB = 512;
struct AffCtl {
    double u[AFF_MAXK];
    double delta[AFF_MAXK];
    int32_t active[AFF_MAXK], iters[AFF_MAXK], just[AFF_MAXK];
    double r_x, r_prev, r_next;
    double s_x, s_prev, s_next;
    double xz_prev[2];
    int32_t n_active, n_just, k_real, it;
};

struct PrParams {
    const uint32_t* in_ptr;
    const uint32_t* in_src;
    const uint32_t* outdeg;
    double* x;
    const double* tab_rd[2];
    double* tab_wr[2];
    const WorkItem* work;
    double* partials;
    double* segpart;
    uint32_t* rowticket;
    PrCtl* ctl;
    const double* x0;
    double d, teleport, eps, tele_n;
    int32_t max_iter, k_topics, world;
    uint32_t sl_nd, cnt_nd, sl_d, cnt_d, seg_edges, n_items;
    uint32_t pos_nd, pos_d;
    const uint32_t* memb;
    const double* tin;
    const double* nz_in;
    uint32_t ts_mask;
    uint32_t zrow;
    const uint32_t* woff;
    uint32_t stagger_div;
    uint32_t stagger_code;
    uint32_t class_order;
    uint32_t n_order;
    double* x_alt;
    AffCtl* aff;
    const double* tele_col;
    const uint32_t* sh_deg;
    uint32_t n_shared;
    uint32_t share;
    uint32_t tab_rows;
};

}

enum PrKernel : int {
    PR_STEP = 0,
    PR_SWEEP = 1,
    PR_SWEEP_N = 2,
};

struct ss_pr {
    ss_graph* g = nullptr;
    PrKernel kernel = PR_SWEEP;
    int gw = 1;
    ss::DevBuf<float> wire_send, wire_recv;
    bool nwave = false;
    int persist_mode = 1;
    bool persist = false;
    int k = 1;
    PrParams prm{};
    unsigned nblocks = 0;
    ss::DevBuf<double> x, tab0, tab1, send, partials, segpart, x0;
    ss::DevBuf<uint32_t> rowticket;
    ss::DevBuf<uint32_t> memb;
    ss::DevBuf<double> tin, nz_in;
    ss::DevBuf<WorkItem> work;
    ss::DevBuf<uint32_t> woff;
    ss::DevBuf<uint32_t> src_shared;
    ss::DevBuf<uint32_t> sh_deg;
    ss::DevBuf<PrCtl> ctl;
    bool begun = false;
    bool need_finalize = false;
    bool finalize_is_begin = false;
};

#pragma GCC visibility push(hidden)
namespace ss {
unsigned begin_blocks(const ss_pr* pr);
void pr_launch_begin(ss_pr* pr, hipStream_t st, unsigned nb);
void pr_launch_step(ss_pr* pr, hipStream_t st);
void pr_launch_finalize(ss_pr* pr, hipStream_t st, int is_begin);
void pr_sweep_launch(ss_pr* pr, hipStream_t st);
int pr_sweep_occupancy(int gw);
void pr_sweep_n_launch(ss_pr* pr, hipStream_t st);
int pr_sweep_n_occupancy(int gw);
void pr_multi_n_launch(ss_pr* pr, hipStream_t st, int n_steps);
int pr_multi_n_occupancy(int gw);
void pr_step_launch(ss_pr* pr, hipStream_t st);
int pr_step_occupancy(int gw);
#ifdef SS_PR_WAVETIME
void pr_dump_wave_times(const ss_pr* pr);
#endif
size_t pr_wire_floats(const ss_pr* pr);
hipError_t pr_wire_alloc(ss_pr* pr);
void pr_wire_pack(ss_pr* pr, hipStream_t st);
void pr_wire_unpack(ss_pr* pr, hipStream_t st);
}
#pragma GCC visibility pop

namespace {
#ifdef SS_PR_WAVETIME
inline FILE* open_dump(const char* name) {
    const char* dir = getenv("SS_PR_WAVETIME_DIR");
    return fopen((std::string(dir && *dir ? dir : ".") + "/" + name).c_str(), "w");
}
#endif
inline int32_t read_ctl(ss_ctx* ctx, const ss_pr* pr, hipStream_t st, const char* what, const PrCtl** out) {
    ctx->pin_used = 0;
    PrCtl* const hp = ctx->pin<PrCtl>();
    if (hipMemcpyAsync(hp, pr->ctl.p, sizeof(PrCtl), hipMemcpyDeviceToHost, st) != hipSuccess) return ctx->fail(SS_ERR_HIP, "%s: status read failed", what);
    SS_TRY(ss::sync_bounded(ctx, st, what));
    *out = hp;
    return SS_OK;
}
}
```

### spaghettisearch_amd/csrc/pr_sweep.hip

```cpp
#include "pr_device.hpp"

#include <algorithm>

namespace {

template <int GW>
__device__ __forceinline__ double tab_at(const double* __restrict__ T, uint32_t row, int t) {
    return *reinterpret_cast<const double*>(reinterpret_cast<const char*>(T) + (size_t)((row * (uint32_t)GW + (uint32_t)t) * 8u));
}


template <int GW, bool TS>
struct SweepCtx {
    const PrParams& p;
    const double* __restrict__ T;
    double* __restrict__ Tw;
    double S, x0;
    bool act;
    int t, gbase, slot;
    double dsum, csum;
};

__device__ __forceinline__ uint32_t turn_fill(uint32_t epos, uint32_t lim) {
    return min((uint32_t)CH, __builtin_elementwise_sub_sat(lim, epos));
}

template <int GW>
__device__ __forceinline__ void idx_turn(const uint32_t* __restrict__ in_src, uint32_t epos, uint32_t n, uint32_t zrow, int t, uint32_t (&src)[CH / GW]) {
#pragma unroll
    for (int r = 0; r < CH / GW; r++) {
        const uint32_t j = (uint32_t)(r * GW + t);
        const uint32_t raw = NT_LOAD(&in_src[j < n ? epos + j : 0u]);
        src[r] = j < n ? (raw & SRC_MASK) : zrow;
    }
}
template <int GW>
__device__ __forceinline__ void gather_turn(const double* __restrict__ T, const uint32_t (&src)[CH / GW], int t, int gbase, double (&v)[CH]) {
#pragma unroll
    for (int j = 0; j < CH; j++) {
        const uint32_t sj = (uint32_t)__shfl((int)src[j / GW], gbase + (j % GW), 64);
        v[j] = tab_at<GW>(T, sj, t);
    }
}

template <int GW, bool TS>
__device__ __forceinline__ void finish_row(SweepCtx<GW, TS>& c, uint32_t lrow, double y, double xo, uint32_t od) {
    const PrParams& p = c.p;
    y += c.x0;
    const size_t xi = (size_t)lrow * GW + c.t;
    double tele = p.teleport;
    if constexpr (TS) tele = teleport_of(p, lrow, c.t);
    double xn = (y + tele) / c.S;
    if (c.act) {
        NT_STORE(xn, &p.x[xi]);
        c.dsum += fabs(xn - xo);
    } else {
        xn = xo;
    }
    if (lrow < p.sl_nd) {
        const double cc = p.d * xn / (double)od;
        NT_STORE(cc, &c.Tw[xi]);
        c.csum += cc;
    }
}

template <int GW, bool TS>
__device__ __forceinline__ void long_rows(SweepCtx<GW, TS>& c, const WorkItem* __restrict__ work, uint32_t i0, uint32_t i1, int lane) {
    constexpr int NS = 64 / GW;
    constexpr uint32_t TW = NS * CH;
    const PrParams& p = c.p;
    if (i0 >= i1) return;
    WorkItem cur = work[i0], nxt = work[i0 + 1];
    uint32_t src_n[CH / GW];
    {
        const uint32_t e0 = cur.beg + (uint32_t)c.slot * CH;
        idx_turn<GW>(p.in_src, e0, turn_fill(e0, cur.end), p.zrow, c.t, src_n);
    }
    for (uint32_t it = i0; it < i1; it++) {
        const WorkItem nn = work[it + 2];
        const uint32_t lrow = cur.row;
        const double xo = NT_LOAD(&p.x[(size_t)lrow * GW + c.t]);
        const uint32_t od = lrow < p.sl_nd ? NT_LOAD(&p.outdeg[lrow]) : 1u;
        const uint32_t turns = (cur.end - cur.beg + TW - 1) / TW;
        const bool more = it + 1 < i1;
        double acc = 0.0;
        for (uint32_t i = 0; i < turns; i++) {
            uint32_t src[CH / GW];
#pragma unroll
            for (int r = 0; r < CH / GW; r++) src[r] = src_n[r];
            const bool last = i + 1 == turns;
            const uint32_t e1 = (last ? nxt.beg : cur.beg + (i + 1) * TW) + (uint32_t)c.slot * CH;
            const uint32_t lim = last ? (more ? nxt.end : 0u) : cur.end;
            idx_turn<GW>(p.in_src, e1, turn_fill(e1, lim), p.zrow, c.t, src_n);
            double v[CH];
            gather_turn<GW>(c.T, src, c.t, c.gbase, v);
#pragma unroll
            for (int j = 0; j < CH; j++) acc += v[j];
        }
        const double y = wave_sum_topic<GW>(acc);
        if (cur.kind == V_ROWW) {
            if (lane < GW) finish_row<GW>(c, lrow, y, xo, od);
        } else {
            if (lane < GW) __hip_atomic_store(&p.segpart[(size_t)(cur.sbase + cur.count) * GW + c.t], y, __ATOMIC_RELAXED, __HIP_MEMORY_SCOPE_AGENT);
            asm volatile("s_waitcnt vmcnt(0)" ::: "memory");
            unsigned prev = 0;
            if (lane == 0) prev = __hip_atomic_fetch_add(&p.rowticket[cur.tix], 1u, __ATOMIC_RELAXED, __HIP_MEMORY_SCOPE_AGENT);
            prev = (unsigned)__builtin_amdgcn_readfirstlane((int)prev);
            if (prev == cur.nseg - 1) {
                if (lane == 0) __hip_atomic_store(&p.rowticket[cur.tix], 0u, __ATOMIC_RELAXED, __HIP_MEMORY_SCOPE_AGENT);
                if (lane < GW) {
                    double ys = 0.0;
                    for (uint32_t q = 0; q < cur.nseg; q++)
                        ys += __hip_atomic_load(&p.segpart[(size_t)(cur.sbase + q) * GW + c.t], __ATOMIC_RELAXED, __HIP_MEMORY_SCOPE_AGENT);
                    finish_row<GW>(c, lrow, ys, xo, od);
                }
            }
        }
        cur = nxt;
        nxt = nn;
    }
}

template <int GW, bool TS>
__device__ __forceinline__ void quad_rows(SweepCtx<GW, TS>& c, const WorkItem* __restrict__ work, uint32_t i0, uint32_t i1) {
    constexpr int NS = 64 / GW;
    const PrParams& p = c.p;
    if (i0 >= i1) return;
    const uint32_t myq = (uint32_t)c.t * NS + (uint32_t)c.slot;
    auto bounds = [&](const WorkItem& w, bool live, uint32_t& bv, uint32_t& ev, uint32_t& ov) __attribute__((always_inline)) {
        const bool have = live && myq < w.count;
        const uint32_t rq = live ? w.row + (have ? myq : 0u) : 0u;
        const uint32_t b = p.in_ptr[rq], e = p.in_ptr[rq + 1];
        bv = b;
        ev = have ? e : b;
        ov = rq < p.sl_nd ? NT_LOAD(&p.outdeg[rq]) : 1u;
    };
    WorkItem cur = work[i0], nxt = work[i0 + 1];
    uint32_t cb, ce, co, nb, ne, no;
    bounds(cur, true, cb, ce, co);
    bounds(nxt, i0 + 1 < i1, nb, ne, no);
    uint32_t it = i0, q = 0, ch = 0;
    uint32_t nq = (cur.count + NS - 1) / NS, nch = cur.nseg;
    uint32_t src_n[CH / GW];
    {
        const uint32_t b0 = (uint32_t)__shfl((int)cb, c.gbase, 64), e0 = (uint32_t)__shfl((int)ce, c.gbase, 64);
        idx_turn<GW>(p.in_src, b0, turn_fill(b0, e0), p.zrow, c.t, src_n);
    }
    double acc = 0.0;
    while (it < i1) {
        uint32_t src[CH / GW];
#pragma unroll
        for (int r = 0; r < CH / GW; r++) src[r] = src_n[r];
        uint32_t qn = q, cn = ch + 1;
        bool cross = false;
        if (cn == nch) {
            cn = 0;
            qn = q + 1;
            if (qn == nq) { qn = 0; cross = true; }
        }
        const bool live_n = !cross || it + 1 < i1;
        {
            const uint32_t b_n = (uint32_t)__shfl((int)(cross ? nb : cb), c.gbase + (int)qn, 64);
            const uint32_t e_n = (uint32_t)__shfl((int)(cross ? ne : ce), c.gbase + (int)qn, 64);
            const uint32_t ep = b_n + cn * CH;
            idx_turn<GW>(p.in_src, ep, live_n ? turn_fill(ep, e_n) : 0u, p.zrow, c.t, src_n);
        }
        const bool ends = ch + 1 == nch;
        const uint32_t lrow = cur.row + q * NS + (uint32_t)c.slot;
        const bool valid = q * NS + (uint32_t)c.slot < cur.count;
        double xo = 0.0;
        if (ends) xo = NT_LOAD(&p.x[(size_t)(valid ? lrow : cur.row) * GW + c.t]);
        double v[CH];
        gather_turn<GW>(c.T, src, c.t, c.gbase, v);
#pragma unroll
        for (int j = 0; j < CH; j++) acc += v[j];
        if (ends) {
            const uint32_t od = (uint32_t)__shfl((int)co, c.gbase + (int)q, 64);
            if (valid) finish_row<GW>(c, lrow, acc, xo, od);
            acc = 0.0;
        }
        q = qn;
        ch = cn;
        if (cross) {
            it++;
            cur = nxt;
            cb = nb; ce = ne; co = no;
            nq = (cur.count + NS - 1) / NS;
            nch = cur.nseg;
            nxt = work[it + 1];
            bounds(nxt, it + 1 < i1, nb, ne, no);
        }
    }
}

template <int GW, int R, bool TS>
__device__ __forceinline__ void deg_rows(SweepCtx<GW, TS>& c, const WorkItem* __restrict__ work, uint32_t i0, uint32_t i1) {
    constexpr int NS = 64 / GW;
    constexpr int DM = CH / R;
    constexpr int IR = CH / GW;
    const PrParams& p = c.p;
    if (i0 >= i1) return;
    auto idx = [&](const WorkItem& w, bool live, uint32_t turn, uint32_t (&src)[IR]) __attribute__((always_inline)) {
        const uint32_t rb = (turn * NS + (uint32_t)c.slot) * R;
#pragma unroll
        for (int r = 0; r < IR; r++) {
            const uint32_t j = (uint32_t)(r * GW + c.t);
            const uint32_t rr = rb + j / DM, u = j % DM;
            const bool ok = live && u < w.nseg && rr < w.count;
            const uint32_t raw = NT_LOAD(&p.in_src[ok ? w.beg + rr * w.nseg + u : 0u]);
            src[r] = ok ? (raw & SRC_MASK) : p.zrow;
        }
    };
    WorkItem cur = work[i0], nxt = work[i0 + 1];
    uint32_t src_n[IR];
    idx(cur, true, 0, src_n);
    for (uint32_t it = i0; it < i1; it++) {
        const WorkItem nn = work[it + 2];
        const uint32_t row0 = cur.row, count = cur.count;
        const uint32_t turns = (count + NS * R - 1) / (NS * R);
        for (uint32_t i = 0; i < turns; i++) {
            uint32_t src[IR];
#pragma unroll
            for (int r = 0; r < IR; r++) src[r] = src_n[r];
            if (i + 1 < turns) idx(cur, true, i + 1, src_n);
            else idx(nxt, it + 1 < i1, 0, src_n);
            const uint32_t rb = (i * NS + (uint32_t)c.slot) * R;
            double xo[R];
#pragma unroll
            for (int r = 0; r < R; r++) xo[r] = NT_LOAD(&p.x[(size_t)(row0 + (rb + r < count ? rb + r : 0u)) * GW + c.t]);
            const uint32_t myr = row0 + (rb + (uint32_t)c.t < count ? rb + (uint32_t)c.t : 0u);
            const uint32_t odv = (c.t < R && myr < p.sl_nd) ? NT_LOAD(&p.outdeg[myr]) : 1u;
            double v[CH];
            gather_turn<GW>(c.T, src, c.t, c.gbase, v);
#pragma unroll
            for (int r = 0; r < R; r++) {
                double y = 0.0;
#pragma unroll
                for (int u = 0; u < DM; u++) y += v[r * DM + u];
                const uint32_t od = (uint32_t)__shfl((int)odv, c.gbase + r, 64);
                if (rb + r < count) finish_row<GW>(c, row0 + rb + r, y, xo[r], od);
            }
        }
        cur = nxt;
        nxt = nn;
    }
}

#ifndef SS_PR_MINW
#define SS_PR_MINW 1
#endif
#ifdef SS_PR_WAVETIME
__device__ unsigned long long g_pr_wt[65536][2];
#endif
template <int GW, bool TS>
__global__ __launch_bounds__(TPB, SS_PR_MINW) void k_pr_sweep(PrParams p) {
    constexpr int NS = 64 / GW;
    PrCtl* ctl = p.ctl;
    if (ctl->n_active == 0) return;
#ifdef SS_PR_WAVETIME
    unsigned long long wt0;
    asm volatile("s_memrealtime %0\n\ts_waitcnt lgkmcnt(0)" : "=s"(wt0));
#endif
    const int sweep = ctl->sweep;
    const int lane = threadIdx.x & 63;
    const uint32_t wave = (uint32_t)__builtin_amdgcn_readfirstlane((int)(threadIdx.x >> 6));
    SweepCtx<GW, TS> c{p, p.tab_rd[sweep & 1], p.tab_wr[sweep & 1], 0.0, 0.0, false, lane % GW, lane - lane % GW, lane / GW, 0.0, 0.0};
    c.S = ctl->S[c.t];
    c.act = ctl->active[c.t] != 0;
    c.x0 = sweep == 0 ? p.x0[c.t] : 0.0;

    if constexpr (!TS) {
        if (p.n_shared) {
            const double xz_out = c.act ? zero_row_rank(p, sweep, c.S, p.x0[c.t]) : ctl->xz[c.t];
            const uint32_t nel = p.n_shared * (uint32_t)GW;
            for (uint32_t i = blockIdx.x * TPB + threadIdx.x; i < nel; i += gridDim.x * TPB)
                c.Tw[(size_t)(p.zrow + 1) * GW + i] = p.d * xz_out / (double)p.sh_deg[i / GW];
        }
    }

    const uint32_t* __restrict__ off = p.woff + (size_t)(blockIdx.x * WAVES + wave) * 8;
    int rot = p.stagger_div ? (int)((blockIdx.x / p.stagger_div) % 6u) : 0;
    if (p.stagger_code) {
        uint32_t cdv = p.stagger_code;
        for (uint32_t r = blockIdx.x / p.stagger_div; r > 0; r--) cdv /= 6u;
        rot = (int)(cdv % 6u);
    }
    for (int s6 = 0; s6 < 6; s6++) {
    const int cls = (int)((p.class_order >> (3 * ((s6 + rot) % 6))) & 7u);
    {
        int ln = lane;
        asm volatile("" : "+v"(ln));
        c.t = ln % GW;
        c.gbase = ln - ln % GW;
        c.slot = ln / GW;
    }
    switch (cls) {
    case 0: long_rows<GW>(c, p.work, off[0], off[1], lane); break;
    case 1: quad_rows<GW>(c, p.work, off[1], off[2]); break;
    case 2: deg_rows<GW, 2>(c, p.work, off[2], off[3]); break;
    case 3: deg_rows<GW, 4>(c, p.work, off[3], off[4]); break;
    case 4: deg_rows<GW, 8>(c, p.work, off[4], off[5]); break;
    default:
    for (uint32_t item = off[5]; item < off[6]; item++) {
        const WorkItem w = p.work[item];
        const bool store = TS || !p.share;
        const bool ts = TS && p.memb && ((p.ts_mask >> c.t) & 1u);
        const double xz_out = c.act ? (ts ? zero_row_rank_ts(p, sweep, c.S, p.x0[c.t], 0.0) : zero_row_rank(p, sweep, c.S, p.x0[c.t])) : ctl->xz[c.t];
        const double xz_inn = ts ? (c.act ? zero_row_rank_ts(p, sweep, c.S, p.x0[c.t], p.tin[c.t]) : ctl->xz_in[c.t]) : xz_out;
        uint32_t od[16];
#pragma unroll
        for (int i = 0; i < 16; i++) {
            const uint32_t rr = (uint32_t)(i * NS + c.slot);
            od[i] = NT_LOAD(&p.outdeg[w.row + (rr < w.count ? rr : 0u)]);
        }
#pragma unroll
        for (int i = 0; i < 16; i++) {
            const uint32_t rr = (uint32_t)(i * NS + c.slot);
            if (rr < w.count) {
                const uint32_t lrow = w.row + rr;
                const double xz = ts && ((p.memb[lrow] >> c.t) & 1u) ? xz_inn : xz_out;
                const double cc = p.d * xz / (double)od[i];
                if (store) NT_STORE(cc, &c.Tw[(size_t)lrow * GW + c.t]);
                c.csum += cc;
            }
        }
    }
    break;
    }
    }
#ifdef SS_PR_WAVETIME
    {
        unsigned long long wt1;
        asm volatile("s_waitcnt vmcnt(0)\n\ts_memrealtime %0\n\ts_waitcnt lgkmcnt(0)" : "=s"(wt1));
        const uint32_t wid = (blockIdx.x * WAVES + wave) & 65535u;
        if (lane == 0) { g_pr_wt[wid][0] = wt0; g_pr_wt[wid][1] = wt1; }
    }
#endif
    block_reduce_and_publish<GW>(p, c.dsum, c.csum, c.Tw, false);
}

template __device__ void begin_caller_context<8, 16>(const PrParams&, double*);

}

namespace ss {
void pr_sweep_launch(ss_pr* pr, hipStream_t st) {
    const bool ts = pr->prm.memb != nullptr;
    if (pr->gw == 8) {
        if (ts) hipLaunchKernelGGL((k_pr_sweep<8, true>), dim3(pr->nblocks), dim3(TPB), 0, st, pr->prm);
        else hipLaunchKernelGGL((k_pr_sweep<8, false>), dim3(pr->nblocks), dim3(TPB), 0, st, pr->prm);
    } else {
        if (ts) hipLaunchKernelGGL((k_pr_sweep<16, true>), dim3(pr->nblocks), dim3(TPB), 0, st, pr->prm);
        else hipLaunchKernelGGL((k_pr_sweep<16, false>), dim3(pr->nblocks), dim3(TPB), 0, st, pr->prm);
    }
}
int pr_sweep_occupancy(int gw) {
    int per_cu = 8;
    if (gw == 8) (void)hipOccupancyMaxActiveBlocksPerMultiprocessor(&per_cu, k_pr_sweep<8, false>, TPB, 0);
    else (void)hipOccupancyMaxActiveBlocksPerMultiprocessor(&per_cu, k_pr_sweep<16, false>, TPB, 0);
    return per_cu;
}

#ifdef SS_PR_WAVETIME
void pr_dump_wave_times(const ss_pr* pr) {
    if (pr->gw < 8) return;
    (void)hipDeviceSynchronize();
    const uint32_t nwv = std::min<uint32_t>(65536u, pr->nblocks * WAVES);
    std::vector<unsigned long long> h((size_t)nwv * 2);
    if (hipMemcpyFromSymbol(h.data(), HIP_SYMBOL(g_pr_wt), h.size() * sizeof(unsigned long long)) != hipSuccess || !nwv) return;
    unsigned long long t0 = ~0ull;
    for (uint32_t w = 0; w < nwv; w++) t0 = std::min(t0, h[2 * w]);
    std::vector<double> st(nwv), en(nwv);
    for (uint32_t w = 0; w < nwv; w++) { st[w] = (double)(h[2 * w] - t0) / 100.0; en[w] = (double)(h[2 * w + 1] - t0) / 100.0; }
    std::sort(st.begin(), st.end()); std::sort(en.begin(), en.end());
    if (FILE* f = open_dump("pr_wt.csv")) {
        fprintf(f, "wave,start_us,end_us\n");
        for (uint32_t w = 0; w < nwv; w++) fprintf(f, "%u,%.2f,%.2f\n", w, (double)(h[2 * w] - t0) / 100.0, (double)(h[2 * w + 1] - t0) / 100.0);
        fclose(f);
    }
    fprintf(stderr, "[pr wavetime] %u waves: start us median %.1f max %.1f | out of items us min %.1f p10 %.1f median %.1f p90 %.1f p99 %.1f max %.1f\n", nwv,
            st[nwv / 2], st[nwv - 1], en[0], en[nwv / 10], en[nwv / 2], en[nwv * 9 / 10], en[(size_t)nwv * 99 / 100], en[nwv - 1]);
}
#endif
}
```

Baseline: 18460.

## Collapse single-in-edge rows sharing a source into twin groups

Rows with exactly one in-edge that share the same source (and out-degree) get identical PageRank values, so they are grouped on the host at create time and each group is computed once by a new V_TWIN work class. Edges and out-degrees are remapped so that readers of any member use the group's representative row, and convergence sums are weighted by group size. This cuts gather and store work per iteration on graphs with many such rows. The cost is an extra host pass, extra device buffers and a remap indirection on readout, and setting a teleport set falls back to rebuilding without twins.

```diff
diff --git a/spaghettisearch_amd/csrc/ctx.hip b/spaghettisearch_amd/csrc/ctx.hip
--- a/spaghettisearch_amd/csrc/ctx.hip
+++ b/spaghettisearch_amd/csrc/ctx.hip
@@ -280,6 +280,7 @@
     "pr.stagger",
     "pr.deal_global",
     "pr.share_zero_rows",
+    "pr.share_twins",
     "pr.item_turns",
     "graph.late_free",
     "pr.trace",
diff --git a/spaghettisearch_amd/csrc/pagerank.hip b/spaghettisearch_amd/csrc/pagerank.hip
--- a/spaghettisearch_amd/csrc/pagerank.hip
+++ b/spaghettisearch_amd/csrc/pagerank.hip
@@ -18,19 +18,33 @@
             w.end = min(in_ptr[w.row + 1], w.beg + SEGW);
             break;
         case V_QUAD:
-        case V_DEG: w.beg = in_ptr[w.row]; w.end = in_ptr[w.row + w.count]; break;
+        case V_DEG:
+        case V_TWIN: w.beg = in_ptr[w.row]; w.end = in_ptr[w.row + w.count]; break;
         default: return;
     }
     work[i] = w;
 }
+
+struct TwinRemap {
+    const uint32_t* new_row;
+    const uint32_t* rank_row;
+    uint32_t row0[2], n[2];
+    uint32_t e0[2];
+};
 
 __global__ __launch_bounds__(TPB) void k_pr_remap_src(const uint32_t* __restrict__ in_src, uint32_t* __restrict__ out, size_t n_edges, uint32_t pos_nd,
                                                       uint32_t cnt_nd, const uint32_t* __restrict__ outdeg, const uint32_t* __restrict__ sh_deg,
-                                                      uint32_t n_shared, uint32_t zrow) {
+                                                      uint32_t n_shared, uint32_t zrow, int share, TwinRemap tw) {
     for (size_t e = (size_t)blockIdx.x * TPB + threadIdx.x; e < n_edges; e += (size_t)gridDim.x * TPB) {
         uint32_t w = NT_LOAD(&in_src[e]);
         const uint32_t s = w & SRC_MASK;
-        if (s >= pos_nd) {
+        size_t eo = e;
+        if (tw.new_row) {
+            if (s - tw.row0[0] < tw.n[0]) w = (w & ~SRC_MASK) | tw.rank_row[s - tw.row0[0]];
+            if (e - tw.e0[0] < tw.n[0]) eo = (size_t)tw.e0[0] + (tw.new_row[e - tw.e0[0]] - tw.row0[0]);
+            else if (e - tw.e0[1] < tw.n[1]) eo = (size_t)tw.e0[1] + (tw.new_row[tw.n[0] + (e - tw.e0[1])] - tw.row0[1]);
+        }
+        if (share && s >= pos_nd) {
             uint32_t row = zrow;
             if (s < cnt_nd && n_shared) {
                 const uint32_t od = outdeg[s];
@@ -43,8 +57,13 @@
             }
             w = (w & ~SRC_MASK) | row;
         }
-        NT_STORE(w, &out[e]);
-    }
+        NT_STORE(w, &out[eo]);
+    }
+}
+__global__ __launch_bounds__(TPB) void k_pr_twin_outdeg(const uint32_t* __restrict__ outdeg, uint32_t* __restrict__ out, uint32_t sl_nd, TwinRemap tw) {
+    const uint32_t i = blockIdx.x * TPB + threadIdx.x;
+    if (i >= sl_nd) return;
+    out[i - tw.row0[0] < tw.n[0] ? tw.new_row[i - tw.row0[0]] : i] = outdeg[i];
 }
 
 template <int GW>
@@ -92,7 +111,7 @@
                           uint32_t sl_nd, uint32_t cnt_nd, uint32_t pos_nd, uint32_t sl_d, uint32_t cnt_d, uint32_t pos_d,
                           uint64_t id0_nd, uint64_t id0_d, int k_topics, uint64_t out_stride,
                           int by_original_id, uint32_t* __restrict__ ids_out, double* __restrict__ out,
-                          const uint32_t* __restrict__ memb, uint32_t ts_mask) {
+                          const uint32_t* __restrict__ memb, uint32_t ts_mask, TwinMap twin) {
     const size_t n_rows = (size_t)cnt_nd + cnt_d;
     size_t i = (size_t)blockIdx.x * blockDim.x + threadIdx.x;
     if (i >= n_rows) return;
@@ -103,8 +122,9 @@
     if (ids_out) ids_out[i] = orig;
     const bool zero = lrow < sl_nd ? lrow >= pos_nd : (lrow - sl_nd) >= pos_d;
     const uint32_t mb = memb ? memb[lrow] & ts_mask : 0u;
+    const uint32_t xrow = twin_rank_row(twin, lrow);
     for (int k = 0; k < k_topics; k++)
-        out[(size_t)k * out_stride + o] = zero ? (((mb >> k) & 1u) ? ctl->xz_in[k] : ctl->xz[k]) : x[(size_t)lrow * GW + k];
+        out[(size_t)k * out_stride + o] = zero ? (((mb >> k) & 1u) ? ctl->xz_in[k] : ctl->xz[k]) : x[(size_t)xrow * GW + k];
 }
 
 __global__ void k_pr_memb(const uint64_t* __restrict__ set_ptr, const uint32_t* __restrict__ set_nodes, int k_topics, uint64_t n_nodes,
@@ -218,7 +238,7 @@
 template <int GW>
 __global__ __launch_bounds__(TPB) void k_pr_read_orig(const double* __restrict__ x, const PrCtl* __restrict__ ctl, const uint32_t* __restrict__ new_id,
                                                       uint64_t n, uint32_t sl_nd, uint32_t pos_nd, uint32_t pos_d, int k_topics,
-                                                      double* __restrict__ out, const uint32_t* __restrict__ memb, uint32_t ts_mask) {
+                                                      double* __restrict__ out, const uint32_t* __restrict__ memb, uint32_t ts_mask, TwinMap twin) {
     const uint64_t v = (uint64_t)blockIdx.x * blockDim.x + threadIdx.x;
     if (v >= n) return;
     const uint32_t lrow = new_id[v];
@@ -226,11 +246,11 @@
     double r[GW];
     if (!zero) {
         if constexpr (GW >= 2) {
-            const double2* const row = reinterpret_cast<const double2*>(x + (size_t)lrow * GW);
+            const double2* const row = reinterpret_cast<const double2*>(x + (size_t)twin_rank_row(twin, lrow) * GW);
 #pragma unroll
             for (int j = 0; j < GW / 2; j++) { const double2 t = row[j]; r[2 * j] = t.x; r[2 * j + 1] = t.y; }
         } else {
-            r[0] = x[lrow];
+            r[0] = x[twin_rank_row(twin, lrow)];
         }
     } else {
         const uint32_t mb = memb ? memb[lrow] & ts_mask : 0u;
@@ -249,14 +269,14 @@
     if (!n_rows) return;
     if (by_orig && g->world == 1 && !ids && stride == g->n) {
         hipLaunchKernelGGL(k_pr_read_orig<GW>, dim3(ss::div_up(g->n, TPB)), dim3(TPB), 0, st, (const double*)pr->x.p, (const PrCtl*)pr->ctl.p,
-                           (const uint32_t*)g->new_id.p, g->n, g->sl_nd, pr->prm.pos_nd, pr->prm.pos_d, pr->k, out, pr->prm.memb, pr->prm.ts_mask);
+                           (const uint32_t*)g->new_id.p, g->n, g->sl_nd, pr->prm.pos_nd, pr->prm.pos_d, pr->k, out, pr->prm.memb, pr->prm.ts_mask, pr->twin_map);
         return;
     }
     hipLaunchKernelGGL(k_pr_read<GW>, dim3(ss::div_up(n_rows, TPB)), dim3(TPB), 0, st, (const double*)pr->x.p,
                        (const PrCtl*)pr->ctl.p, (const uint32_t*)g->old_id.p, g->sl_nd, g->cnt_nd, pr->prm.pos_nd, g->sl_d, g->cnt_d,
                        pr->prm.pos_d,
                        (uint64_t)g->rank * g->sl_nd, g->nd_int + (uint64_t)g->rank * g->sl_d, pr->k, stride, by_orig, ids, out,
-                       pr->prm.memb, pr->prm.ts_mask);
+                       pr->prm.memb, pr->prm.ts_mask, pr->twin_map);
 }
 
 #define SS_GW_DISPATCH(gw, fn, ...)          \
@@ -436,12 +456,7 @@
 }
 #endif
 
-}
-
-extern "C" {
-
-int32_t ss_pr_create(ss_graph* g, double damping, double eps, int32_t max_iter, int32_t k_topics,
-                     const int32_t* n_topic, ss_pr** out) {
+int32_t pr_create(ss_graph* g, double damping, double eps, int32_t max_iter, int32_t k_topics, const int32_t* n_topic, bool allow_twins, ss_pr** out) {
     if (!g) return SS_ERR_INVALID;
     ss_ctx* ctx = g->ctx;
     std::lock_guard<std::recursive_mutex> lk(ctx->mu);
@@ -457,6 +472,7 @@
     std::unique_ptr<ss_pr> guard(pr);
     pr->g = g;
     pr->k = k_topics;
+    std::copy(n_topic, n_topic + k_topics, pr->n_topic);
     pick_kernel(ctx, pr, k_topics, g->nd_int);
     const int GW = pr->gw;
     const bool vitems = pr->kernel != PR_STEP;
@@ -475,7 +491,49 @@
 
     const auto tc0 = t_now();
     const PlanOptions opt = plan_options(ctx, pr, n_local);
-    Cut cut = cut_items(g->h_indeg_nd, g->h_indeg_d, g->sl_nd, GI, pr->nwave, opt);
+    bool twins = allow_twins && GW >= 8 && g->world == 1 && ctx->opt("pr.affine", 0) == 0 && ctx->opt("pr.share_twins", 1) != 0;
+    TwinPlan tp;
+    TwinRemap twr{};
+    if (twins) {
+        const uint32_t a[2] = {g->h_indeg_nd.first_at_most(1), g->h_indeg_d.first_at_most(1)};
+        const uint32_t row0[2] = {a[0], g->sl_nd + a[1]};
+        const uint32_t n[2] = {g->h_indeg_nd.first_at_most(0) - a[0], g->h_indeg_d.first_at_most(0) - a[1]};
+        if ((uint64_t)n[0] + n[1] >= TWIN_MIN) {
+            const auto tt0 = t_now();
+            struct Pin { ss_ctx* c; void* p = nullptr; size_t cap = 0; ~Pin() { c->pin_free(p, cap); } } pin{ctx};
+            const size_t words = 2 + 2 * (size_t)n[0] + n[1];
+            pin.p = ctx->pin_alloc(words * sizeof(uint32_t), &pin.cap);
+            if (!pin.p) return ctx->fail(SS_ERR_OOM, "ss_pr_create: no pinned host memory for %zu words of the rows with one in-edge", words);
+            uint32_t* const h = static_cast<uint32_t*>(pin.p);
+            h[0] = h[1] = 0;
+            for (int r = 0; r < 2; r++) {
+                if (!n[r]) continue;
+                SS_HIP(ctx, hipMemcpyAsync(h + r, g->in_ptr.p + row0[r], sizeof(uint32_t), hipMemcpyDeviceToHost, st));
+            }
+            SS_HIP(ctx, hipStreamSynchronize(st));
+            const uint32_t e0[2] = {h[0], h[1]};
+            uint32_t* const hs[2] = {h + 2, h + 2 + 2 * (size_t)n[0]};
+            uint32_t* const ho = h + 2 + n[0];
+            for (int r = 0; r < 2; r++) {
+                if (!n[r]) continue;
+                if ((uint64_t)e0[r] + n[r] > g->e_local) return ctx->fail(SS_ERR_STATE, "ss_pr_create: the rows with one in-edge end behind the edge list");
+                SS_HIP(ctx, hipMemcpyAsync(hs[r], g->in_src.p + e0[r], (size_t)n[r] * sizeof(uint32_t), hipMemcpyDeviceToHost, st));
+            }
+            if (n[0]) { SS_HIP(ctx, hipMemcpyAsync(ho, g->outdeg.p + row0[0], (size_t)n[0] * sizeof(uint32_t), hipMemcpyDeviceToHost, st)); }
+            SS_HIP(ctx, hipStreamSynchronize(st));
+            for (int r = 0; r < 2; r++)
+                for (uint32_t i = 0; i < n[r]; i++) hs[r][i] &= SRC_MASK;
+            const auto tt1 = t_now();
+            const uint32_t* const srcs[2] = {hs[0], hs[1]};
+            const uint32_t* const ods[2] = {ho, nullptr};
+            tp = plan_twin_groups(srcs, ods, row0, n);
+            if (trace) fprintf(stderr, "[pr trace]   twin groups: %u + %u rows with one in-edge -> %u + %u single rows, %u + %u collapsed groups (fetch %.3f ms, host %.3f ms)\n",
+                               n[0], n[1], tp.n_single[0], tp.n_single[1], tp.n_group[0], tp.n_group[1], t_ms(tt0, tt1), t_ms(tt1, t_now()));
+            for (int r = 0; r < 2; r++) { twr.row0[r] = row0[r]; twr.n[r] = n[r]; twr.e0[r] = e0[r]; }
+        }
+        twins = tp.any();
+    }
+    Cut cut = cut_items(g->h_indeg_nd, g->h_indeg_d, g->sl_nd, GI, pr->nwave, opt, twins ? &tp : nullptr);
     const uint32_t n_tail = g->cnt_nd - cut.pos_nd;
     struct PinGuard { ss_ctx* c; void* p = nullptr; size_t cap = 0; ~PinGuard() { c->pin_free(p, cap); } } tail_od{ctx};
     if (share && n_tail == 0) {
@@ -520,13 +578,28 @@
         SS_TRY(alloc_tables(pr, st, (size_t)sh.table_rows));
         SS_HIP(ctx, pr->sh_deg.alloc(sh.deg.size()));
         SS_HIP(ctx, hipMemcpyAsync(pr->sh_deg.p, sh.deg.data(), sh.deg.size() * sizeof(uint32_t), hipMemcpyHostToDevice, st));
+        if (trace) fprintf(stderr, "[pr trace]   shared rows: %u rows without in-edges -> %zu shared rows (host %.3f ms), table %llu rows\n", n_tail, sh.deg.size(),
+                           t_ms(ts0, ts1), (unsigned long long)sh.table_rows);
+    }
+    if (twins) {
+        SS_HIP(ctx, pr->tw_new_row.alloc(tp.new_row.size()));
+        SS_HIP(ctx, pr->tw_rank_row.alloc(tp.rank_row.size()));
+        SS_HIP(ctx, pr->tw_cnt.alloc(tp.count.size()));
+        SS_HIP(ctx, pr->tw_outdeg.alloc(g->sl_nd));
+        SS_HIP(ctx, hipMemcpyAsync(pr->tw_new_row.p, tp.new_row.data(), tp.new_row.size() * sizeof(uint32_t), hipMemcpyHostToDevice, st));
+        SS_HIP(ctx, hipMemcpyAsync(pr->tw_rank_row.p, tp.rank_row.data(), tp.rank_row.size() * sizeof(uint32_t), hipMemcpyHostToDevice, st));
+        SS_HIP(ctx, hipMemcpyAsync(pr->tw_cnt.p, tp.count.data(), tp.count.size() * sizeof(uint32_t), hipMemcpyHostToDevice, st));
+        twr.new_row = pr->tw_new_row.p;
+        twr.rank_row = pr->tw_rank_row.p;
+        if (g->sl_nd)
+            hipLaunchKernelGGL(k_pr_twin_outdeg, dim3(ss::div_up(g->sl_nd, TPB)), dim3(TPB), 0, st, (const uint32_t*)g->outdeg.p, pr->tw_outdeg.p, g->sl_nd, twr);
+    }
+    if (share || twins) {
         SS_HIP(ctx, pr->src_shared.alloc(g->e_local));
         if (g->e_local)
             hipLaunchKernelGGL(k_pr_remap_src, dim3((unsigned)std::min<uint64_t>(ss::div_up(g->e_local, TPB), (uint64_t)ctx->cu_count * 16)), dim3(TPB), 0, st,
                                (const uint32_t*)g->in_src.p, pr->src_shared.p, (size_t)g->e_local, cut.pos_nd, g->cnt_nd, (const uint32_t*)g->outdeg.p,
-                               (const uint32_t*)pr->sh_deg.p, (uint32_t)sh.deg.size(), sh.zrow);
-        if (trace) fprintf(stderr, "[pr trace]   shared rows: %u rows without in-edges -> %zu shared rows (host %.3f ms), table %llu rows\n", n_tail, sh.deg.size(),
-                           t_ms(ts0, ts1), (unsigned long long)sh.table_rows);
+                               (const uint32_t*)pr->sh_deg.p, (uint32_t)sh.deg.size(), sh.zrow, share ? 1 : 0, twr);
     }
     SS_HIP(ctx, pr->partials.alloc(((size_t)std::max(pr->nblocks, ss::begin_blocks(pr)) + 8) * 2 * GW));
     SS_HIP(ctx, pr->segpart.alloc((size_t)std::max(cut.nsegs, 1u) * GW));
@@ -559,10 +632,26 @@
         p.zrow = sh.zrow;
         p.tab_rows = cut.pos_nd;
     }
+    if (twins) {
+        PrParams& p = pr->prm;
+        p.in_src = pr->src_shared.p;
+        p.outdeg = pr->tw_outdeg.p;
+        p.twin_cnt = pr->tw_cnt.p;
+        pr->twin_map = TwinMap{pr->tw_rank_row.p, {twr.row0[0], twr.row0[1]}, {twr.n[0], twr.n[1]}};
+    }
     if (trace) trace_plan(pr, items, *woff);
     g->users++;
     *out = guard.release();
     return SS_OK;
+}
+
+}
+
+extern "C" {
+
+int32_t ss_pr_create(ss_graph* g, double damping, double eps, int32_t max_iter, int32_t k_topics,
+                     const int32_t* n_topic, ss_pr** out) {
+    return pr_create(g, damping, eps, max_iter, k_topics, n_topic, true, out);
 }
 
 int32_t ss_pr_set_teleport(ss_pr* pr, const uint64_t* set_ptr, const uint32_t* set_nodes) {
@@ -579,6 +668,14 @@
     }
     const ss_graph* g = pr->g;
     const int K = pr->k;
+    if (pr->twin_map.rank_row) {
+        ss_pr* fresh = nullptr;
+        SS_TRY(pr_create(pr->g, p.d, p.eps, p.max_iter, K, pr->n_topic, false, &fresh));
+        std::unique_ptr<ss_pr> owner(fresh);
+        SS_HIP(ctx, hipStreamSynchronize(st));
+        *pr = std::move(*fresh);
+        pr->g->users--;
+    }
     SS_TRY(unshare_rows(pr, st));
     std::vector<uint64_t> h_ptr(K + 1);
     SS_HIP(ctx, ss::copy_in(ctx->stream, h_ptr.data(), set_ptr, (K + 1) * sizeof(uint64_t)));
diff --git a/spaghettisearch_amd/csrc/pr_plan.hpp b/spaghettisearch_amd/csrc/pr_plan.hpp
--- a/spaghettisearch_amd/csrc/pr_plan.hpp
+++ b/spaghettisearch_amd/csrc/pr_plan.hpp
@@ -18,7 +18,8 @@
                   V_ROWW = 9,
                   V_QUAD = 10,
                   V_DEG = 11,
-                  V_ZERO = 12 };
+                  V_ZERO = 12,
+                  V_TWIN = 13 };
 
 struct WorkItem {
     uint32_t kind;
@@ -47,7 +48,7 @@
 
 struct PlanScratch {
     std::vector<WorkItem> seg, rwg, wav, grp, zer;
-    std::vector<WorkItem> vseg, vroww, vquad, vdeg[3], vzero;
+    std::vector<WorkItem> vseg, vroww, vquad, vdeg[3], vzero, vtwin;
     std::vector<WorkItem> items, dealt;
     std::vector<double> cost, load;
     std::vector<uint32_t> owner, by_load, idx, order, bucket, woff, cnt;
@@ -63,10 +64,89 @@
     uint32_t nsegs = 0, nmulti = 0;
     uint32_t seg_edges = 0;
     uint32_t pos_nd = 0, pos_d = 0;
-    uint32_t vbeg[7] = {0};
-};
-
-inline Cut cut_items(const ss::SortedDegrees& nd, const ss::SortedDegrees& d, uint32_t sl_nd, int gw, bool lane_rows, const PlanOptions& opt) {
+    uint32_t vbeg[8] = {0};
+};
+constexpr int N_VCLASS = 7;
+
+constexpr uint32_t TWIN_MIN = 2;
+struct TwinPlan {
+    uint32_t row0[2] = {0, 0}, n[2] = {0, 0};
+    uint32_t n_single[2] = {0, 0}, n_group[2] = {0, 0};
+    std::vector<uint32_t> new_row;
+    std::vector<uint32_t> rank_row;
+    std::vector<uint32_t> count;
+    bool any() const { return n_group[0] + n_group[1] > 0; }
+    uint32_t rank_row_of(uint32_t lrow) const {
+        if (lrow - row0[0] < n[0]) return rank_row[lrow - row0[0]];
+        if (lrow - row0[1] < n[1]) return rank_row[n[0] + (lrow - row0[1])];
+        return lrow;
+    }
+};
+inline TwinPlan plan_twin_groups(const uint32_t* const src[2], const uint32_t* const od[2], const uint32_t row0[2], const uint32_t n[2]) {
+    TwinPlan tp;
+    tp.new_row.resize((size_t)n[0] + n[1]);
+    tp.rank_row.resize((size_t)n[0] + n[1]);
+    std::vector<uint32_t> bucket, order;
+    size_t base = 0;
+    for (int r = 0; r < 2; r++) {
+        tp.row0[r] = row0[r];
+        tp.n[r] = n[r];
+        const uint32_t nr = n[r];
+        const uint32_t* s = src[r];
+        const uint32_t* o = od[r];
+        order.resize(nr);
+        uint32_t hi = 0;
+        for (uint32_t i = 0; i < nr; i++) hi = std::max(hi, s[i]);
+        const auto by_od = [&](uint32_t a, uint32_t b) { return o[a] < o[b]; };
+        if (nr && (uint64_t)hi <= 4 * (uint64_t)nr + 65536) {
+            bucket.assign((size_t)hi + 2, 0u);
+            for (uint32_t i = 0; i < nr; i++) bucket[(size_t)s[i] + 1]++;
+            for (size_t v = 0; v <= hi; v++) bucket[v + 1] += bucket[v];
+            for (uint32_t i = 0; i < nr; i++) order[bucket[s[i]]++] = i;
+        } else {
+            for (uint32_t i = 0; i < nr; i++) order[i] = i;
+            std::stable_sort(order.begin(), order.end(), [&](uint32_t a, uint32_t b) { return s[a] < s[b]; });
+        }
+        for (uint32_t i = 0; i < nr && o;) {
+            uint32_t j = i + 1;
+            while (j < nr && s[order[j]] == s[order[i]]) j++;
+            if (j - i > 1) std::stable_sort(order.begin() + i, order.begin() + j, by_od);
+            i = j;
+        }
+        const auto group_end = [&](uint32_t a) {
+            uint32_t b = a + 1;
+            while (b < nr && s[order[b]] == s[order[a]] && (!o || o[order[b]] == o[order[a]])) b++;
+            return b;
+        };
+        uint32_t n_single = 0, n_group = 0;
+        for (uint32_t a = 0; a < nr;) {
+            const uint32_t b = group_end(a);
+            if (b - a >= TWIN_MIN) n_group++; else n_single += b - a;
+            a = b;
+        }
+        tp.n_single[r] = n_single;
+        tp.n_group[r] = n_group;
+        uint32_t at_single = row0[r], at_rep = row0[r] + n_single, at_member = row0[r] + n_single + n_group;
+        for (uint32_t a = 0; a < nr;) {
+            const uint32_t b = group_end(a);
+            if (b - a >= TWIN_MIN) {
+                tp.count.push_back(b - a);
+                tp.new_row[base + order[a]] = at_rep;
+                for (uint32_t q = a + 1; q < b; q++) tp.new_row[base + order[q]] = at_member++;
+                for (uint32_t q = a; q < b; q++) tp.rank_row[base + order[q]] = at_rep;
+                at_rep++;
+            } else {
+                for (uint32_t q = a; q < b; q++) tp.new_row[base + order[q]] = tp.rank_row[base + order[q]] = at_single++;
+            }
+            a = b;
+        }
+        base += nr;
+    }
+    return tp;
+}
+
+inline Cut cut_items(const ss::SortedDegrees& nd, const ss::SortedDegrees& d, uint32_t sl_nd, int gw, bool lane_rows, const PlanOptions& opt,
+                     const TwinPlan* tw = nullptr) {
     PlanScratch& s = plan_scratch();
     Cut cut{s.items};
     uint32_t& nsegs = cut.nsegs;
@@ -76,9 +156,10 @@
     const uint32_t T_WAVE = 2 * NSLOT;
     const uint32_t seg_edges = cut.seg_edges = 128 * NSLOT;
     auto &seg = s.seg, &rwg = s.rwg, &wav = s.wav, &grp = s.grp, &zer = s.zer;
-    auto &vseg = s.vseg, &vroww = s.vroww, &vquad = s.vquad, &vzero = s.vzero;
+    auto &vseg = s.vseg, &vroww = s.vroww, &vquad = s.vquad, &vzero = s.vzero, &vtwin = s.vtwin;
     auto& vdeg = s.vdeg;
-    for (auto* v : {&seg, &rwg, &wav, &grp, &zer, &vseg, &vroww, &vquad, &vdeg[0], &vdeg[1], &vdeg[2], &vzero}) v->clear();
+    for (auto* v : {&seg, &rwg, &wav, &grp, &zer, &vseg, &vroww, &vquad, &vdeg[0], &vdeg[1], &vdeg[2], &vzero, &vtwin}) v->clear();
+    uint32_t twin_base = 0;
     auto emit_v = [&](const ss::SortedDegrees& deg, uint32_t row0, bool non_dangling, uint32_t& n_pos) {
         const uint32_t cnt = (uint32_t)deg.size();
         const uint32_t T_MULTI = 4096, T_DEG = 8;
@@ -121,7 +202,15 @@
             const uint32_t R = D <= 2 ? 8 : D <= 4 ? 4 : 2;
             const uint32_t per_item = lane_rows ? 64u * item_turns : NSLOT * R * item_turns;
             auto& out = vdeg[R == 2 ? 0 : R == 4 ? 1 : 2];
-            for (uint32_t o = 0; o < run; o += per_item) out.push_back({V_DEG, row0 + r + o, std::min(per_item, run - o), D, 0, 0});
+            const int tr = non_dangling ? 0 : 1;
+            const bool twins = tw && D == 1 && tw->n[tr] == run && tw->row0[tr] == row0 + r;
+            const uint32_t plain = twins ? tw->n_single[tr] : run;
+            for (uint32_t o = 0; o < plain; o += per_item) out.push_back({V_DEG, row0 + r + o, std::min(per_item, plain - o), D, 0, 0});
+            if (twins) {
+                const uint32_t ng = tw->n_group[tr], per_twin = NSLOT * 8 * item_turns;
+                for (uint32_t o = 0; o < ng; o += per_twin) vtwin.push_back({V_TWIN, row0 + r + plain + o, std::min(per_twin, ng - o), 1, twin_base + o, 0});
+                twin_base += ng;
+            }
             r += run;
         }
         n_pos = r;
@@ -177,7 +266,12 @@
     vbeg[5] = (uint32_t)items.size();
     items.insert(items.end(), vzero.begin(), vzero.end());
     vbeg[6] = (uint32_t)items.size();
-    if (items.empty()) items.push_back({W_ZERO, 0, 0, 0, 0, 0});
+    items.insert(items.end(), vtwin.begin(), vtwin.end());
+    vbeg[7] = (uint32_t)items.size();
+    if (items.empty()) {
+        items.push_back({W_ZERO, 0, 0, 0, 0, 0});
+        vbeg[6] = vbeg[7] = 1;
+    }
     return cut;
 }
 
@@ -210,6 +304,7 @@
                 turns = (double)plan_div_up(w.count, NS * R) * (R == 8 ? 2.5 : R == 4 ? 1.7 : 1.3);
                 break;
             }
+            case V_TWIN: turns = (double)plan_div_up(w.count, NS * 8u) * 1.5; break;
             default: turns = 0.5; break;
         }
         cost[i] = turns + 1.0;
@@ -236,8 +331,8 @@
         bucket.assign(NB + 1, 0u);
         order.resize(n_items);
         size_t c0 = 0;
-        for (int kcls = 0; kcls < (deal_mode == 2 ? 6 : 1); kcls++) {
-            const size_t c1 = deal_mode == 2 ? (kcls < 5 ? std::min<size_t>(cut.vbeg[kcls + 1], n_items) : n_items) : n_items;
+        for (int kcls = 0; kcls < (deal_mode == 2 ? N_VCLASS : 1); kcls++) {
+            const size_t c1 = deal_mode == 2 ? (kcls < N_VCLASS - 1 ? std::min<size_t>(cut.vbeg[kcls + 1], n_items) : n_items) : n_items;
             if (kcls) std::fill(bucket.begin(), bucket.end(), 0u);
             for (size_t i = c0; i < c1; i++) bucket[bkey(i) + 1]++;
             for (uint32_t b = 0; b < NB; b++) bucket[b + 1] += bucket[b];
@@ -281,8 +376,8 @@
     auto &woff = s.woff, &cnt = s.cnt;
     woff.assign((size_t)nw * 8, 0);
     cnt.assign((size_t)nw * 8, 0);
-    for (int k = 0; k < 6; k++) {
-        const size_t i1 = k < 5 ? std::min<size_t>(cut.vbeg[k + 1], items.size()) : items.size();
+    for (int k = 0; k < N_VCLASS; k++) {
+        const size_t i1 = k < N_VCLASS - 1 ? std::min<size_t>(cut.vbeg[k + 1], items.size()) : items.size();
         for (size_t i = std::min<size_t>(cut.vbeg[k], i1); i < i1; i++) { owner[i] = owner[i] * 8 + (uint32_t)k; cnt[owner[i]]++; }
     }
     uint32_t run_off = 0;
diff --git a/spaghettisearch_amd/csrc/pr_state.hpp b/spaghettisearch_amd/csrc/pr_state.hpp
--- a/spaghettisearch_amd/csrc/pr_state.hpp
+++ b/spaghettisearch_amd/csrc/pr_state.hpp
@@ -74,7 +74,19 @@
     uint32_t n_shared;
     uint32_t share;
     uint32_t tab_rows;
+    const uint32_t* twin_cnt;
 };
+
+struct TwinMap {
+    const uint32_t* rank_row;
+    uint32_t row0[2], n[2];
+};
+__device__ __forceinline__ uint32_t twin_rank_row(const TwinMap& m, uint32_t lrow) {
+    if (!m.rank_row) return lrow;
+    if (lrow - m.row0[0] < m.n[0]) return m.rank_row[lrow - m.row0[0]];
+    if (lrow - m.row0[1] < m.n[1]) return m.rank_row[m.n[0] + (lrow - m.row0[1])];
+    return lrow;
+}
 
 }
 
@@ -103,6 +115,9 @@
     ss::DevBuf<uint32_t> woff;
     ss::DevBuf<uint32_t> src_shared;
     ss::DevBuf<uint32_t> sh_deg;
+    ss::DevBuf<uint32_t> tw_new_row, tw_rank_row, tw_cnt, tw_outdeg;
+    TwinMap twin_map{};
+    int32_t n_topic[MAXK] = {};
     ss::DevBuf<PrCtl> ctl;
     bool begun = false;
     bool need_finalize = false;
diff --git a/spaghettisearch_amd/csrc/pr_sweep.hip b/spaghettisearch_amd/csrc/pr_sweep.hip
--- a/spaghettisearch_amd/csrc/pr_sweep.hip
+++ b/spaghettisearch_amd/csrc/pr_sweep.hip
@@ -246,6 +246,68 @@
     }
 }
 
+template <int GW>
+__device__ __forceinline__ void twin_rows(SweepCtx<GW, false>& c, const WorkItem* __restrict__ work, uint32_t i0, uint32_t i1) {
+    constexpr int NS = 64 / GW;
+    constexpr int R = 8;
+    const PrParams& p = c.p;
+    if (i0 >= i1) return;
+    auto idx = [&](const WorkItem& w, bool live, uint32_t turn, uint32_t& src, uint32_t& odv, uint32_t& cntv) __attribute__((always_inline)) {
+        const uint32_t rr = (turn * NS + (uint32_t)c.slot) * R + (uint32_t)c.t;
+        const bool ok = live && c.t < R && rr < w.count;
+        const uint32_t raw = NT_LOAD(&p.in_src[ok ? w.beg + rr : 0u]);
+        src = ok ? (raw & SRC_MASK) : p.zrow;
+        const uint32_t lrow = w.row + (ok ? rr : 0u);
+        const uint32_t od = NT_LOAD(&p.outdeg[ok && lrow < p.sl_nd ? lrow : 0u]);
+        odv = ok && lrow < p.sl_nd ? od : 1u;
+        const uint32_t cn = NT_LOAD(&p.twin_cnt[ok ? w.sbase + rr : 0u]);
+        cntv = ok ? cn : 0u;
+    };
+    WorkItem cur = work[i0], nxt = work[i0 + 1];
+    uint32_t src_n, od_n, cnt_n;
+    idx(cur, true, 0, src_n, od_n, cnt_n);
+    for (uint32_t it = i0; it < i1; it++) {
+        const WorkItem nn = work[it + 2];
+        const uint32_t row0 = cur.row, count = cur.count;
+        const uint32_t turns = (count + NS * R - 1) / (NS * R);
+        for (uint32_t i = 0; i < turns; i++) {
+            const uint32_t src = src_n, odv = od_n, cntv = cnt_n;
+            if (i + 1 < turns) idx(cur, true, i + 1, src_n, od_n, cnt_n);
+            else idx(nxt, it + 1 < i1, 0, src_n, od_n, cnt_n);
+            const uint32_t rb = (i * NS + (uint32_t)c.slot) * R;
+            double xo[R], v[R];
+#pragma unroll
+            for (int r = 0; r < R; r++) xo[r] = NT_LOAD(&p.x[(size_t)(row0 + (rb + r < count ? rb + r : 0u)) * GW + c.t]);
+#pragma unroll
+            for (int r = 0; r < R; r++) v[r] = tab_at<GW>(c.T, (uint32_t)__shfl((int)src, c.gbase + r, 64), c.t);
+#pragma unroll
+            for (int r = 0; r < R; r++) {
+                const uint32_t od = (uint32_t)__shfl((int)odv, c.gbase + r, 64);
+                const double members = (double)(uint32_t)__shfl((int)cntv, c.gbase + r, 64);
+                if (rb + r < count) {
+                    const uint32_t lrow = row0 + rb + r;
+                    const size_t xi = (size_t)lrow * GW + c.t;
+                    const double y = 0.0 + v[r] + c.x0;
+                    double xn = (y + p.teleport) / c.S;
+                    if (c.act) {
+                        NT_STORE(xn, &p.x[xi]);
+                        c.dsum += members * fabs(xn - xo[r]);
+                    } else {
+                        xn = xo[r];
+                    }
+                    if (lrow < p.sl_nd) {
+                        const double cc = p.d * xn / (double)od;
+                        NT_STORE(cc, &c.Tw[xi]);
+                        c.csum += members * cc;
+                    }
+                }
+            }
+        }
+        cur = nxt;
+        nxt = nn;
+    }
+}
+
 #ifndef SS_PR_MINW
 #define SS_PR_MINW 1
 #endif
@@ -285,6 +347,14 @@
         for (uint32_t r = blockIdx.x / p.stagger_div; r > 0; r--) cdv /= 6u;
         rot = (int)(cdv % 6u);
     }
+    if constexpr (!TS) {
+        int ln = lane;
+        asm volatile("" : "+v"(ln));
+        c.t = ln % GW;
+        c.gbase = ln - ln % GW;
+        c.slot = ln / GW;
+        twin_rows<GW>(c, p.work, off[6], off[7]);
+    }
     for (int s6 = 0; s6 < 6; s6++) {
     const int cls = (int)((p.class_order >> (3 * ((s6 + rot) % 6))) & 7u);
     {
```

Measured after the change: 18690, median of 6. 1.2% higher.
